# westlake-repl/Adapter4Rec

Measured on NVIDIA B200. Metric: train user-sequences/s (SASRec + BERT-base LoRA r=8 adapter-tuning step: fwd+bwd+allreduce+Adam), higher is better.
Workload: dtype bf16

## Files before the change

### adapter4rec_b200/csrc/attention_mid.cu

```cuda
#include "a4r_common.cuh"
#include "mma_sync.cuh"

namespace {

constexpr int DH = 64;
constexpr int WARPS = 8;
constexpr int LMAX = 256;

A4R_DEVICE uint32_t toff(int row, int chunk) { return static_cast<uint32_t>(row * 128 + (((chunk ^ row) & 7) << 4)); }

struct MidParams {
  const __nv_bfloat16* qkv;
  __nv_bfloat16* out;
  const __nv_bfloat16* dout;
  const void* mask;
  float* lse;
  const __nv_bfloat16* ctx;
  int64_t ld_qkv, ld_out, mask_ld;
  int N, L, Lp, heads;
  int mask_dtype;
  float scale, mask_neg;
};

A4R_DEVICE void load_rows(uint8_t* tile, const __nv_bfloat16* g, int64_t ld, int L, int Lp) {
  const uint32_t base = smem_u32(tile);
  for (int i = threadIdx.x; i < Lp * 8; i += WARPS * 32) {
    const int row = i >> 3, ch = i & 7;
    const bool ok = row < L;
    const __nv_bfloat16* src = g + (ok ? static_cast<int64_t>(row) * ld + ch * 8 : 0);
    const int sz = ok ? 16 : 0;
    asm volatile("cp.async.cg.shared.global [%0], [%1], 16, %2;" ::"r"(base + toff(row, ch)), "l"(src), "r"(sz) : "memory");
  }
}
A4R_DEVICE void cp_async_wait_all() { asm volatile("cp.async.wait_all;" ::: "memory"); }

A4R_DEVICE void lda(uint32_t (&a)[4], uint32_t base, int m0, int k0, int lane) {
  const int mi = lane >> 3, r = lane & 7;
  ldsm_x4(a, base + toff(m0 + r + ((mi & 1) << 3), (k0 >> 3) + (mi >> 1)));
}
A4R_DEVICE void ldb_nk(uint32_t (&b)[4], uint32_t base, int n0, int k0, int lane) {
  const int mi = lane >> 3, r = lane & 7;
  ldsm_x4(b, base + toff(n0 + r + ((mi >> 1) << 3), (k0 >> 3) + (mi & 1)));
}
A4R_DEVICE void ldb_kn(uint32_t (&b)[4], uint32_t base, int n0, int k0, int lane) {
  const int mi = lane >> 3, r = lane & 7;
  ldsm_x4_t(b, base + toff(k0 + r + ((mi & 1) << 3), (n0 >> 3) + (mi >> 1)));
}
A4R_DEVICE void c2a(uint32_t (&a)[4], const float (&c0)[4], const float (&c1)[4]) {
  a[0] = pack_bf16x2(c0[0], c0[1]);
  a[1] = pack_bf16x2(c0[2], c0[3]);
  a[2] = pack_bf16x2(c1[0], c1[1]);
  a[3] = pack_bf16x2(c1[2], c1[3]);
}

A4R_DEVICE bool key_ok(const MidParams& p, int n, int j) {
  if (j >= p.L) return false;
  if (p.mask_dtype == 1) return reinterpret_cast<const int64_t*>(p.mask)[static_cast<int64_t>(n) * p.mask_ld + j] != 0;
  if (p.mask_dtype == 2) return reinterpret_cast<const float*>(p.mask)[static_cast<int64_t>(n) * p.mask_ld + j] != 0.0f;
  return true;
}

A4R_DEVICE void score_block(float (&s)[8][4], const uint32_t (&qa)[4][4], uint32_t sK, int key0, int lane, int nv) {
#pragma unroll
  for (int nt = 0; nt < 8; ++nt)
#pragma unroll
    for (int e = 0; e < 4; ++e) s[nt][e] = 0.0f;
#pragma unroll
  for (int ks = 0; ks < 4; ++ks) {
#pragma unroll
    for (int np = 0; np < 4; ++np) {
      if (np < nv) {
        uint32_t b[4];
        ldb_nk(b, sK, key0 + np * 16, ks * 16, lane);
        const uint32_t b0[2] = {b[0], b[1]}, b1[2] = {b[2], b[3]};
        mma_bf16_16816(s[np * 2], qa[ks], b0);
        mma_bf16_16816(s[np * 2 + 1], qa[ks], b1);
      }
    }
  }
}

A4R_DEVICE void mask_block(float (&s)[8][4], const MidParams& p, const uint32_t* kvalid, int key0, int lane) {
  const int t = lane & 3;
#pragma unroll
  for (int nt = 0; nt < 8; ++nt)
#pragma unroll
    for (int e = 0; e < 4; ++e) {
      const int j = key0 + nt * 8 + 2 * t + (e & 1);
      float v = s[nt][e] * p.scale;
      const bool valid = (kvalid[j >> 5] >> (j & 31)) & 1u;
      if (!valid) v += p.mask_neg;
      if (j >= p.L) v = -INFINITY;
      s[nt][e] = v;
    }
}

__global__ void __launch_bounds__(WARPS * 32, 2) attn_mid_fwd_kernel(const MidParams p) {
  extern __shared__ __align__(128) uint8_t sm_mid[];
  __shared__ uint32_t kvalid[LMAX / 32];
  const int warp = threadIdx.x >> 5, lane = threadIdx.x & 31;
  const int g = lane >> 2, t = lane & 3;
  const int tile_bytes = p.Lp * 128;
  uint8_t *tQ = sm_mid, *tK = sm_mid + tile_bytes, *tV = sm_mid + 2 * tile_bytes;
  const uint32_t sQ = smem_u32(tQ), sK = smem_u32(tK), sV = smem_u32(tV);
  const int64_t Hd = static_cast<int64_t>(p.heads) * DH;
  for (int w = blockIdx.x; w < p.N * p.heads; w += gridDim.x) {
    const int n = w / p.heads, h = w % p.heads;
    const __nv_bfloat16* q = p.qkv + static_cast<int64_t>(n) * p.L * p.ld_qkv + h * DH;
    __syncthreads();
    load_rows(tQ, q, p.ld_qkv, p.L, p.Lp);
    load_rows(tK, q + Hd, p.ld_qkv, p.L, p.Lp);
    load_rows(tV, q + 2 * Hd, p.ld_qkv, p.L, p.Lp);
    if (threadIdx.x < LMAX / 32) {
      uint32_t bits = 0;
      for (int j = 0; j < 32; ++j) bits |= (key_ok(p, n, threadIdx.x * 32 + j) ? 1u : 0u) << j;
      kvalid[threadIdx.x] = bits;
    }
    cp_async_wait_all();
    __syncthreads();
    for (int m0 = warp * 16; m0 < p.Lp && m0 < ((p.L + 15) & ~15); m0 += WARPS * 16) {
      uint32_t qa[4][4];
#pragma unroll
      for (int ks = 0; ks < 4; ++ks) lda(qa[ks], sQ, m0, ks * 16, lane);
      float o[8][4];
#pragma unroll
      for (int nt = 0; nt < 8; ++nt)
#pragma unroll
        for (int e = 0; e < 4; ++e) o[nt][e] = 0.0f;
      float mx[2] = {-INFINITY, -INFINITY}, sum[2] = {0.0f, 0.0f};
      for (int key0 = 0; key0 < p.Lp; key0 += 64) {
        float s[8][4];
        const int nv = min(4, (p.L - key0 + 15) >> 4);
        score_block(s, qa, sK, key0, lane, nv);
        mask_block(s, p, kvalid, key0, lane);
#pragma unroll
        for (int hh = 0; hh < 2; ++hh) {
          float bm = -INFINITY;
#pragma unroll
          for (int nt = 0; nt < 8; ++nt) bm = fmaxf(bm, fmaxf(s[nt][hh * 2], s[nt][hh * 2 + 1]));
          bm = fmaxf(bm, __shfl_xor_sync(0xffffffffu, bm, 1));
          bm = fmaxf(bm, __shfl_xor_sync(0xffffffffu, bm, 2));
          const float nm = fmaxf(mx[hh], bm);
          const float corr = (mx[hh] == -INFINITY) ? 0.0f : __expf(mx[hh] - nm);
          mx[hh] = nm;
          float bs = 0.0f;
#pragma unroll
          for (int nt = 0; nt < 8; ++nt)
#pragma unroll
            for (int e = 0; e < 2; ++e) {
              const float ex = (nm == -INFINITY || (nt >> 1) >= nv) ? 0.0f : __expf(s[nt][hh * 2 + e] - nm);
              s[nt][hh * 2 + e] = ex;
              bs += ex;
            }
          bs += __shfl_xor_sync(0xffffffffu, bs, 1);
          bs += __shfl_xor_sync(0xffffffffu, bs, 2);
          sum[hh] = sum[hh] * corr + bs;
#pragma unroll
          for (int nt = 0; nt < 8; ++nt) {
            o[nt][hh * 2] *= corr;
            o[nt][hh * 2 + 1] *= corr;
          }
        }
#pragma unroll
        for (int ks = 0; ks < 4; ++ks) {
          if (ks < nv) {
            uint32_t a[4];
            c2a(a, s[2 * ks], s[2 * ks + 1]);
#pragma unroll
            for (int np = 0; np < 4; ++np) {
              uint32_t b[4];
              ldb_kn(b, sV, np * 16, key0 + ks * 16, lane);
              const uint32_t b0[2] = {b[0], b[1]}, b1[2] = {b[2], b[3]};
              mma_bf16_16816(o[np * 2], a, b0);
              mma_bf16_16816(o[np * 2 + 1], a, b1);
            }
          }
        }
      }
      const float inv0 = 1.0f / sum[0], inv1 = 1.0f / sum[1];
      __nv_bfloat16* op = p.out + (static_cast<int64_t>(n) * p.L) * p.ld_out + h * DH;
      const int r0 = m0 + g, r1 = m0 + g + 8;
      if (p.lse != nullptr && t == 0) {
        if (r0 < p.L) p.lse[(static_cast<int64_t>(n) * p.L + r0) * p.heads + h] = mx[0] + __logf(sum[0]);
        if (r1 < p.L) p.lse[(static_cast<int64_t>(n) * p.L + r1) * p.heads + h] = mx[1] + __logf(sum[1]);
      }
#pragma unroll
      for (int nt = 0; nt < 8; ++nt) {
        const int col = nt * 8 + 2 * t;
        if (r0 < p.L) *reinterpret_cast<uint32_t*>(op + static_cast<int64_t>(r0) * p.ld_out + col) = pack_bf16x2(o[nt][0] * inv0, o[nt][1] * inv0);
        if (r1 < p.L) *reinterpret_cast<uint32_t*>(op + static_cast<int64_t>(r1) * p.ld_out + col) = pack_bf16x2(o[nt][2] * inv1, o[nt][3] * inv1);
      }
    }
  }
}

__global__ void __launch_bounds__(WARPS * 32) attn_mid_bwd_kernel(const MidParams p) {
  extern __shared__ __align__(128) uint8_t sm_mid[];
  __shared__ uint32_t kvalid[LMAX / 32];
  __shared__ float s_lse[LMAX], s_delta[LMAX];
  const int warp = threadIdx.x >> 5, lane = threadIdx.x & 31;
  const int g = lane >> 2, t = lane & 3;
  const int tile_bytes = p.Lp * 128;
  uint8_t *tQ = sm_mid, *tK = tQ + tile_bytes, *tV = tK + tile_bytes, *tdO = tV + tile_bytes;
  const uint32_t sQ = smem_u32(tQ), sK = smem_u32(tK), sV = smem_u32(tV), sdO = smem_u32(tdO);
  const int64_t Hd = static_cast<int64_t>(p.heads) * DH;
  const int Lq = (p.L + 15) & ~15;
  for (int w = blockIdx.x; w < p.N * p.heads; w += gridDim.x) {
    const int n = w / p.heads, h = w % p.heads;
    const __nv_bfloat16* q = p.qkv + static_cast<int64_t>(n) * p.L * p.ld_qkv + h * DH;
    __nv_bfloat16* dq = p.out + static_cast<int64_t>(n) * p.L * p.ld_qkv + h * DH;
    __syncthreads();
    load_rows(tQ, q, p.ld_qkv, p.L, p.Lp);
    load_rows(tK, q + Hd, p.ld_qkv, p.L, p.Lp);
    load_rows(tV, q + 2 * Hd, p.ld_qkv, p.L, p.Lp);
    load_rows(tdO, p.dout + static_cast<int64_t>(n) * p.L * p.ld_out + h * DH, p.ld_out, p.L, p.Lp);
    if (threadIdx.x < LMAX / 32) {
      uint32_t bits = 0;
      for (int j = 0; j < 32; ++j) bits |= (key_ok(p, n, threadIdx.x * 32 + j) ? 1u : 0u) << j;
      kvalid[threadIdx.x] = bits;
    }
    cp_async_wait_all();
    __syncthreads();
    for (int r = threadIdx.x; r < p.Lp; r += WARPS * 32)
      s_lse[r] = r < p.L ? p.lse[(static_cast<int64_t>(n) * p.L + r) * p.heads + h] : 0.0f;
    for (int i = threadIdx.x; i < p.Lp * 8; i += WARPS * 32) {
      const int r = i >> 3, ch = i & 7;
      float d = 0.0f;
      if (r < p.L) {
        const int64_t grow = static_cast<int64_t>(n) * p.L + r;
        const uint4 ov = ld_nc_v4(p.ctx + grow * p.ld_out + h * DH + ch * 8);
        const uint4 dv4 = *reinterpret_cast<const uint4*>(tdO + toff(r, ch));
        const uint32_t ow[4] = {ov.x, ov.y, ov.z, ov.w}, dw[4] = {dv4.x, dv4.y, dv4.z, dv4.w};
#pragma unroll
        for (int e = 0; e < 4; ++e) {
          const float2 a = unpack_bf16x2(ow[e]), b = unpack_bf16x2(dw[e]);
          d += a.x * b.x + a.y * b.y;
        }
      }
      d += __shfl_xor_sync(0xffffffffu, d, 1);
      d += __shfl_xor_sync(0xffffffffu, d, 2);
      d += __shfl_xor_sync(0xffffffffu, d, 4);
      if (ch == 0) s_delta[r] = d;
    }
    __syncthreads();
    for (int m0 = warp * 16; m0 < Lq; m0 += WARPS * 16) {
      uint32_t qa[4][4], da[4][4];
#pragma unroll
      for (int ks = 0; ks < 4; ++ks) {
        lda(qa[ks], sQ, m0, ks * 16, lane);
        lda(da[ks], sdO, m0, ks * 16, lane);
      }
      const float lse[2] = {s_lse[m0 + g], s_lse[m0 + g + 8]};
      const float delta[2] = {s_delta[m0 + g], s_delta[m0 + g + 8]};
      float acc[8][4];
#pragma unroll
      for (int nt = 0; nt < 8; ++nt)
#pragma unroll
        for (int e = 0; e < 4; ++e) acc[nt][e] = 0.0f;
      for (int key0 = 0; key0 < p.Lp; key0 += 64) {
        float s[8][4], dp[8][4];
        const int nv = min(4, (p.L - key0 + 15) >> 4);
        score_block(s, qa, sK, key0, lane, nv);
        mask_block(s, p, kvalid, key0, lane);
        score_block(dp, da, sV, key0, lane, nv);
#pragma unroll
        for (int nt = 0; nt < 8; ++nt)
          if ((nt >> 1) < nv) {
#pragma unroll
            for (int e = 0; e < 4; ++e)
              s[nt][e] = __expf(s[nt][e] - lse[e >> 1]) * (dp[nt][e] - delta[e >> 1]) * p.scale;
          }
#pragma unroll
        for (int ks = 0; ks < 4; ++ks) {
          if (ks < nv) {
            uint32_t a[4];
            c2a(a, s[2 * ks], s[2 * ks + 1]);
#pragma unroll
            for (int np = 0; np < 4; ++np) {
              uint32_t b[4];
              ldb_kn(b, sK, np * 16, key0 + ks * 16, lane);
              const uint32_t b0[2] = {b[0], b[1]}, b1[2] = {b[2], b[3]};
              mma_bf16_16816(acc[np * 2], a, b0);
              mma_bf16_16816(acc[np * 2 + 1], a, b1);
            }
          }
        }
      }
      const int r0 = m0 + g, r1 = m0 + g + 8;
#pragma unroll
      for (int nt = 0; nt < 8; ++nt) {
        const int col = nt * 8 + 2 * t;
        if (r0 < p.L) *reinterpret_cast<uint32_t*>(dq + static_cast<int64_t>(r0) * p.ld_qkv + col) = pack_bf16x2(acc[nt][0], acc[nt][1]);
        if (r1 < p.L) *reinterpret_cast<uint32_t*>(dq + static_cast<int64_t>(r1) * p.ld_qkv + col) = pack_bf16x2(acc[nt][2], acc[nt][3]);
      }
    }
    for (int j0 = warp * 16; j0 < Lq; j0 += WARPS * 16) {
      uint32_t ka[4][4], va[4][4];
#pragma unroll
      for (int ks = 0; ks < 4; ++ks) {
        lda(ka[ks], sK, j0, ks * 16, lane);
        lda(va[ks], sV, j0, ks * 16, lane);
      }
      const int jr[2] = {j0 + g, j0 + g + 8};
      bool kv[2];
#pragma unroll
      for (int hh = 0; hh < 2; ++hh) kv[hh] = (kvalid[jr[hh] >> 5] >> (jr[hh] & 31)) & 1u;
      float dk[8][4], dv[8][4];
#pragma unroll
      for (int nt = 0; nt < 8; ++nt)
#pragma unroll
        for (int e = 0; e < 4; ++e) dk[nt][e] = dv[nt][e] = 0.0f;
      for (int i0 = 0; i0 < p.Lp; i0 += 64) {
        float st[8][4], dpt[8][4];
        const int nv = min(4, (p.L - i0 + 15) >> 4);
        score_block(st, ka, sQ, i0, lane, nv);
        score_block(dpt, va, sdO, i0, lane, nv);
#pragma unroll
        for (int nt = 0; nt < 8; ++nt)
#pragma unroll
          for (int e = 0; e < 4; ++e) {
            const int i = i0 + nt * 8 + 2 * t + (e & 1);
            const int hh = e >> 1;
            float v = st[nt][e] * p.scale;
            if (!kv[hh]) v += p.mask_neg;
            float pr = 0.0f, ds = 0.0f;
            if (jr[hh] < p.L && i < p.L) {
              pr = __expf(v - s_lse[i]);
              ds = pr * (dpt[nt][e] - s_delta[i]) * p.scale;
            }
            st[nt][e] = pr;
            dpt[nt][e] = ds;
          }
#pragma unroll
        for (int ks = 0; ks < 4; ++ks) {
          if (ks >= nv) continue;
          uint32_t pa[4], sa[4];
          c2a(pa, st[2 * ks], st[2 * ks + 1]);
          c2a(sa, dpt[2 * ks], dpt[2 * ks + 1]);
#pragma unroll
          for (int np = 0; np < 4; ++np) {
            uint32_t b[4], c[4];
            ldb_kn(b, sQ, np * 16, i0 + ks * 16, lane);
            ldb_kn(c, sdO, np * 16, i0 + ks * 16, lane);
            const uint32_t b0[2] = {b[0], b[1]}, b1[2] = {b[2], b[3]};
            const uint32_t c0[2] = {c[0], c[1]}, c1[2] = {c[2], c[3]};
            mma_bf16_16816(dk[np * 2], sa, b0);
            mma_bf16_16816(dk[np * 2 + 1], sa, b1);
            mma_bf16_16816(dv[np * 2], pa, c0);
            mma_bf16_16816(dv[np * 2 + 1], pa, c1);
          }
        }
      }
#pragma unroll
      for (int nt = 0; nt < 8; ++nt) {
        const int col = nt * 8 + 2 * t;
#pragma unroll
        for (int hh = 0; hh < 2; ++hh) {
          if (jr[hh] < p.L) {
            __nv_bfloat16* row = dq + static_cast<int64_t>(jr[hh]) * p.ld_qkv + col;
            *reinterpret_cast<uint32_t*>(row + Hd) = pack_bf16x2(dk[nt][hh * 2], dk[nt][hh * 2 + 1]);
            *reinterpret_cast<uint32_t*>(row + 2 * Hd) = pack_bf16x2(dv[nt][hh * 2], dv[nt][hh * 2 + 1]);
          }
        }
      }
    }
  }
}

constexpr float LOG2E = 1.4426950408889634f;


int check_mid(const a4r_attn_args* a) {
  A4R_CHECK_ARG(a != nullptr && a->qkv && a->out, "attention_mid: NULL pointer");
  A4R_CHECK_ARG(a->L >= 1 && a->L <= LMAX, "attention_mid: L must be in [1,256] (got %lld)", (long long)a->L);
  A4R_CHECK_ARG(a->head_dim == DH, "attention_mid: head_dim must be 64");
  A4R_CHECK_ARG(a->causal == 0, "attention_mid: causal masking is not supported (use the short-sequence kernel)");
  A4R_CHECK_ARG(a->dropout_p == 0.0f, "attention_mid: probability dropout is not implemented (ViT uses p = 0)");
  A4R_CHECK_ARG(a->heads >= 1 && a->N >= 0, "attention_mid: bad heads/N");
  A4R_CHECK_ARG(a->ld_qkv >= 3 * a->heads * DH && a->ld_qkv % 8 == 0 && a->ld_out >= a->heads * DH && a->ld_out % 8 == 0,
                "attention_mid: bad leading dimensions");
  A4R_CHECK_ARG(a4r_aligned16(a->qkv) && a4r_aligned16(a->out), "attention_mid: pointers must be 16B aligned");
  A4R_CHECK_ARG(a->mask_dtype >= 0 && a->mask_dtype <= 2, "attention_mid: mask_dtype must be 0,1,2");
  if (a->mask_dtype != 0) A4R_CHECK_ARG(a->mask != nullptr && a->mask_ld >= a->L, "attention_mid: bad mask");
  return a4r_device_check();
}

MidParams mid_params(const a4r_attn_args* a) {
  MidParams p;
  p.qkv = static_cast<const __nv_bfloat16*>(a->qkv);
  p.out = static_cast<__nv_bfloat16*>(a->out);
  p.dout = static_cast<const __nv_bfloat16*>(a->dout);
  p.mask = a->mask;
  p.lse = a->lse;
  p.ctx = static_cast<const __nv_bfloat16*>(a->ctx);
  p.ld_qkv = a->ld_qkv;
  p.ld_out = a->ld_out;
  p.mask_ld = a->mask_ld;
  p.N = static_cast<int>(a->N);
  p.L = static_cast<int>(a->L);
  p.Lp = (p.L + 63) & ~63;
  p.heads = static_cast<int>(a->heads);
  p.mask_dtype = a->mask_dtype;
  p.scale = a->scale;
  p.mask_neg = a->mask_neg;
  return p;
}

}

int a4r_attn_vit_tc_fwd(const a4r_attn_args* a, cudaStream_t stream);
int a4r_attn_vit_tc_bwd(const a4r_attn_args* a, cudaStream_t stream);

extern "C" int a4r_attn_mid_fwd(const a4r_attn_args* a, a4r_stream_t stream) {
  int rc = check_mid(a);
  if (rc != A4R_OK) return rc;
  if (a->N == 0) return A4R_OK;
  if (a->mask_dtype == 0) return a4r_attn_vit_tc_fwd(a, static_cast<cudaStream_t>(stream));
  const MidParams p = mid_params(a);
  const int smem = 3 * p.Lp * 128;
  A4R_CUDA_OK(cudaFuncSetAttribute(attn_mid_fwd_kernel, cudaFuncAttributeMaxDynamicSharedMemorySize, 3 * LMAX * 128));
  int64_t blocks = static_cast<int64_t>(p.N) * p.heads;
  const int64_t cap = static_cast<int64_t>(a4r_num_sms()) * 4;
  if (blocks > cap) blocks = cap;
  attn_mid_fwd_kernel<<<static_cast<int>(blocks), WARPS * 32, smem, static_cast<cudaStream_t>(stream)>>>(p);
  A4R_LAUNCH_OK();
  a4r_count_launch(1);
  return A4R_OK;
}

extern "C" int a4r_attn_mid_bwd(const a4r_attn_args* a, a4r_stream_t stream) {
  int rc = check_mid(a);
  if (rc != A4R_OK) return rc;
  A4R_CHECK_ARG(a->dout != nullptr && a4r_aligned16(a->dout), "attention_mid bwd: dout missing or unaligned");
  A4R_CHECK_ARG(a->lse != nullptr && a->ctx != nullptr, "attention_mid bwd: needs the forward's lse and ctx outputs");
  if (a->N == 0) return A4R_OK;
  if (a->mask_dtype == 0) return a4r_attn_vit_tc_bwd(a, static_cast<cudaStream_t>(stream));
  const MidParams p = mid_params(a);
  const int smem = 4 * p.Lp * 128;
  A4R_CUDA_OK(cudaFuncSetAttribute(attn_mid_bwd_kernel, cudaFuncAttributeMaxDynamicSharedMemorySize, 4 * LMAX * 128));
  int64_t blocks = static_cast<int64_t>(p.N) * p.heads;
  const int64_t cap = static_cast<int64_t>(a4r_num_sms()) * 2;
  if (blocks > cap) blocks = cap;
  attn_mid_bwd_kernel<<<static_cast<int>(blocks), WARPS * 32, smem, static_cast<cudaStream_t>(stream)>>>(p);
  A4R_LAUNCH_OK();
  a4r_count_launch(1);
  return A4R_OK;
}
```

### adapter4rec_b200/csrc/attention_small.cu

```cuda
#include "a4r_common.cuh"
#include "mma_sync.cuh"

namespace {

constexpr int LP = 32;
constexpr int WARPS_PER_CTA = 4;

struct AttnParams {
  const __nv_bfloat16* qkv;
  __nv_bfloat16* out;
  const __nv_bfloat16* dout;
  const void* mask;
  int64_t ld_qkv, ld_out, mask_ld;
  int N, L, heads;
  int mask_dtype;
  const int32_t* cu_seqlens;
  int causal;
  float scale, mask_neg;
  uint32_t drop_thr16;
  float drop_scale;
  uint64_t drop_seed, drop_offset;
};

A4R_DEVICE void prob_dropout(float (&s)[2][4][4], const AttnParams& p, int n, int h, int lane) {
  const int g = lane >> 2, t = lane & 3;
  const uint64_t base = p.drop_offset + (static_cast<uint64_t>(n) * p.heads + h) * (32 * 8);
  const uint64_t seed = rng_seed(p.drop_seed);
#pragma unroll
  for (int mt = 0; mt < 2; ++mt)
#pragma unroll
    for (int hh = 0; hh < 2; ++hh) {
      const int i = mt * 16 + hh * 8 + g;
#pragma unroll
      for (int np = 0; np < 2; ++np) {
        const uint64_t r = rng64(seed, base + static_cast<uint64_t>(i) * 8 + np * 4 + t);
#pragma unroll
        for (int q = 0; q < 2; ++q)
#pragma unroll
          for (int e = 0; e < 2; ++e) {
            float& x = s[mt][np * 2 + q][hh * 2 + e];
            x = rng_keep(r, q * 2 + e, p.drop_thr16) ? x * p.drop_scale : 0.0f;
          }
      }
    }
}

template <int COLS>
struct Tile {
  static constexpr int kChunks = COLS / 8;
  static constexpr int kBytes = LP * COLS * 2;
  A4R_DEVICE static uint32_t off(int row, int chunk) {
    const int x = COLS == 64 ? row : (row >> 1);
    return static_cast<uint32_t>(row * COLS * 2 + (((chunk ^ x) & (kChunks - 1)) << 4));
  }
};

template <int COLS>
A4R_DEVICE void load_a(uint32_t (&a)[4], uint32_t base, int m0, int k0, int lane) {
  const int mi = lane >> 3, r = lane & 7;
  const int row = m0 + r + ((mi & 1) << 3);
  const int chunk = (k0 >> 3) + (mi >> 1);
  ldsm_x4(a, base + Tile<COLS>::off(row, chunk));
}
template <int COLS>
A4R_DEVICE void load_a_t(uint32_t (&a)[4], uint32_t base, int m0, int k0, int lane) {
  const int mi = lane >> 3, r = lane & 7;
  const int row = k0 + r + ((mi >> 1) << 3);
  const int chunk = (m0 >> 3) + (mi & 1);
  ldsm_x4_t(a, base + Tile<COLS>::off(row, chunk));
}
template <int COLS>
A4R_DEVICE void load_b_nk(uint32_t (&b)[4], uint32_t base, int n0, int k0, int lane) {
  const int mi = lane >> 3, r = lane & 7;
  const int row = n0 + r + ((mi >> 1) << 3);
  const int chunk = (k0 >> 3) + (mi & 1);
  ldsm_x4(b, base + Tile<COLS>::off(row, chunk));
}
template <int COLS>
A4R_DEVICE void load_b_kn(uint32_t (&b)[4], uint32_t base, int n0, int k0, int lane) {
  const int mi = lane >> 3, r = lane & 7;
  const int row = k0 + r + ((mi & 1) << 3);
  const int chunk = (n0 >> 3) + (mi >> 1);
  ldsm_x4_t(b, base + Tile<COLS>::off(row, chunk));
}

template <int DH>
A4R_DEVICE void load_tile(uint8_t* tile, const __nv_bfloat16* g, int64_t ld, int L, int lane) {
  constexpr int CH = DH / 8;
  const uint32_t base = smem_u32(tile);
#pragma unroll
  for (int i = lane; i < LP * CH; i += 32) {
    const int row = i / CH, ch = i % CH;
    const bool ok = row < L;
    const __nv_bfloat16* src = g + (ok ? static_cast<int64_t>(row) * ld + ch * 8 : 0);
    const int sz = ok ? 16 : 0;
    asm volatile("cp.async.cg.shared.global [%0], [%1], 16, %2;" ::"r"(base + Tile<DH>::off(row, ch)), "l"(src), "r"(sz)
                 : "memory");
  }
}
A4R_DEVICE void cp_async_wait_all() { asm volatile("cp.async.wait_all;" ::: "memory"); }
template <int DH>
A4R_DEVICE void store_tile(const uint8_t* tile, __nv_bfloat16* g, int64_t ld, int L, int lane) {
  constexpr int CH = DH / 8;
#pragma unroll
  for (int i = lane; i < LP * CH; i += 32) {
    const int row = i / CH, ch = i % CH;
    if (row < L) st_na_v4(g + static_cast<int64_t>(row) * ld + ch * 8, *reinterpret_cast<const uint4*>(tile + Tile<DH>::off(row, ch)));
  }
}
template <int COLS, int NT>
A4R_DEVICE void acc_to_tile(uint8_t* tile, const float (&acc)[2][NT][4], float s0a, float s0b, float s1a, float s1b, int lane) {
  const int g = lane >> 2, t = lane & 3;
#pragma unroll
  for (int mt = 0; mt < 2; ++mt) {
    const float sa = mt == 0 ? s0a : s1a, sb = mt == 0 ? s0b : s1b;
#pragma unroll
    for (int nt = 0; nt < NT; ++nt) {
      const int r0 = mt * 16 + g, col = nt * 8 + 2 * t;
      *reinterpret_cast<uint32_t*>(tile + Tile<COLS>::off(r0, col >> 3) + (col & 7) * 2) =
          pack_bf16x2(acc[mt][nt][0] * sa, acc[mt][nt][1] * sa);
      *reinterpret_cast<uint32_t*>(tile + Tile<COLS>::off(r0 + 8, col >> 3) + (col & 7) * 2) =
          pack_bf16x2(acc[mt][nt][2] * sb, acc[mt][nt][3] * sb);
    }
  }
}

struct SeqSpan {
  int64_t row0, mask0;
  int L;
};
A4R_DEVICE SeqSpan seq_span(const AttnParams& p, int n) {
  SeqSpan s;
  if (p.cu_seqlens != nullptr) {
    const int a = __ldg(p.cu_seqlens + n), b = __ldg(p.cu_seqlens + n + 1);
    s.row0 = a, s.mask0 = a, s.L = b - a;
  } else {
    s.row0 = static_cast<int64_t>(n) * p.L, s.mask0 = static_cast<int64_t>(n) * p.mask_ld, s.L = p.L;
  }
  return s;
}
A4R_DEVICE bool key_valid(const AttnParams& p, const SeqSpan& sq, int j) {
  if (p.mask_dtype == 1) return reinterpret_cast<const int64_t*>(p.mask)[sq.mask0 + j] != 0;
  if (p.mask_dtype == 2) return reinterpret_cast<const float*>(p.mask)[sq.mask0 + j] != 0.0f;
  return true;
}

template <int DH>
A4R_DEVICE void scores_softmax(float (&s)[2][4][4], uint32_t sQ, uint32_t sK, const AttnParams& p, int L, int lane,
                               uint32_t keymask_bits) {
#pragma unroll
  for (int mt = 0; mt < 2; ++mt)
#pragma unroll
    for (int nt = 0; nt < 4; ++nt)
#pragma unroll
      for (int e = 0; e < 4; ++e) s[mt][nt][e] = 0.0f;
#pragma unroll
  for (int k0 = 0; k0 < DH; k0 += 16) {
    uint32_t a0[4], a1[4];
    load_a<DH>(a0, sQ, 0, k0, lane);
    load_a<DH>(a1, sQ, 16, k0, lane);
#pragma unroll
    for (int np = 0; np < 2; ++np) {
      uint32_t b[4];
      load_b_nk<DH>(b, sK, np * 16, k0, lane);
      const uint32_t b0[2] = {b[0], b[1]}, b1[2] = {b[2], b[3]};
      mma_bf16_16816(s[0][np * 2], a0, b0);
      mma_bf16_16816(s[0][np * 2 + 1], a0, b1);
      mma_bf16_16816(s[1][np * 2], a1, b0);
      mma_bf16_16816(s[1][np * 2 + 1], a1, b1);
    }
  }
  const int g = lane >> 2, t = lane & 3;
  float colneg[4][2];
#pragma unroll
  for (int nt = 0; nt < 4; ++nt)
#pragma unroll
    for (int e = 0; e < 2; ++e) {
      const int j = nt * 8 + 2 * t + e;
      colneg[nt][e] = j >= L ? -INFINITY : (((keymask_bits >> j) & 1u) ? 0.0f : p.mask_neg);
    }
#pragma unroll
  for (int mt = 0; mt < 2; ++mt) {
#pragma unroll
    for (int h = 0; h < 2; ++h) {
      const int i = mt * 16 + h * 8 + g;
      float mx = -INFINITY;
#pragma unroll
      for (int nt = 0; nt < 4; ++nt)
#pragma unroll
        for (int e = 0; e < 2; ++e) {
          float v = fmaf(s[mt][nt][h * 2 + e], p.scale, colneg[nt][e]);
          if (p.causal && nt * 8 + 2 * t + e > i && colneg[nt][e] == 0.0f) v += p.mask_neg;
          s[mt][nt][h * 2 + e] = v;
          mx = fmaxf(mx, v);
        }
      mx = fmaxf(mx, __shfl_xor_sync(0xffffffffu, mx, 1));
      mx = fmaxf(mx, __shfl_xor_sync(0xffffffffu, mx, 2));
      float sum = 0.0f;
#pragma unroll
      for (int nt = 0; nt < 4; ++nt)
#pragma unroll
        for (int e = 0; e < 2; ++e) {
          const float ex = __expf(s[mt][nt][h * 2 + e] - mx);
          s[mt][nt][h * 2 + e] = ex;
          sum += ex;
        }
      sum += __shfl_xor_sync(0xffffffffu, sum, 1);
      sum += __shfl_xor_sync(0xffffffffu, sum, 2);
      const float inv = 1.0f / sum;
#pragma unroll
      for (int nt = 0; nt < 4; ++nt)
#pragma unroll
        for (int e = 0; e < 2; ++e) s[mt][nt][h * 2 + e] *= inv;
    }
  }
}

A4R_DEVICE uint32_t build_keymask(const AttnParams& p, const SeqSpan& sq, int lane) {
  const bool ok = lane < sq.L ? key_valid(p, sq, lane) : false;
  return __ballot_sync(0xffffffffu, ok);
}

A4R_DEVICE void acc_to_a(uint32_t (&a)[4], const float (&c0)[4], const float (&c1)[4]) {
  a[0] = pack_bf16x2(c0[0], c0[1]);
  a[1] = pack_bf16x2(c0[2], c0[3]);
  a[2] = pack_bf16x2(c1[0], c1[1]);
  a[3] = pack_bf16x2(c1[2], c1[3]);
}

template <int DH>
__global__ void __launch_bounds__(WARPS_PER_CTA * 32, 3) attn_fwd_kernel(const AttnParams p) {
  extern __shared__ __align__(128) uint8_t smem_attn[];
  constexpr int TB = Tile<DH>::kBytes;
  const int warp = threadIdx.x >> 5, lane = threadIdx.x & 31;
  uint8_t* my = smem_attn + warp * 3 * TB;
  const int64_t total = static_cast<int64_t>(p.N) * p.heads;
  for (int64_t w = static_cast<int64_t>(blockIdx.x) * WARPS_PER_CTA + warp; w < total;
       w += static_cast<int64_t>(gridDim.x) * WARPS_PER_CTA) {
    const int n = static_cast<int>(w / p.heads), h = static_cast<int>(w % p.heads);
    const int64_t Hd = static_cast<int64_t>(p.heads) * DH;
    const SeqSpan sq = seq_span(p, n);
    const __nv_bfloat16* q = p.qkv + sq.row0 * p.ld_qkv + h * DH;
    load_tile<DH>(my, q, p.ld_qkv, sq.L, lane);
    load_tile<DH>(my + TB, q + Hd, p.ld_qkv, sq.L, lane);
    load_tile<DH>(my + 2 * TB, q + 2 * Hd, p.ld_qkv, sq.L, lane);
    const uint32_t km = build_keymask(p, sq, lane);
    cp_async_wait_all();
    __syncwarp();
    const uint32_t sQ = smem_u32(my), sK = sQ + TB, sV = sK + TB;
    float s[2][4][4];
    scores_softmax<DH>(s, sQ, sK, p, sq.L, lane, km);
    if (p.drop_thr16 != 0) prob_dropout(s, p, n, h, lane);
    float o[2][DH / 8][4];
#pragma unroll
    for (int mt = 0; mt < 2; ++mt)
#pragma unroll
      for (int nt = 0; nt < DH / 8; ++nt)
#pragma unroll
        for (int e = 0; e < 4; ++e) o[mt][nt][e] = 0.0f;
#pragma unroll
    for (int ks = 0; ks < 2; ++ks) {
      uint32_t a0[4], a1[4];
      acc_to_a(a0, s[0][2 * ks], s[0][2 * ks + 1]);
      acc_to_a(a1, s[1][2 * ks], s[1][2 * ks + 1]);
#pragma unroll
      for (int np = 0; np < DH / 16; ++np) {
        uint32_t b[4];
        load_b_kn<DH>(b, sV, np * 16, ks * 16, lane);
        const uint32_t b0[2] = {b[0], b[1]}, b1[2] = {b[2], b[3]};
        mma_bf16_16816(o[0][np * 2], a0, b0);
        mma_bf16_16816(o[0][np * 2 + 1], a0, b1);
        mma_bf16_16816(o[1][np * 2], a1, b0);
        mma_bf16_16816(o[1][np * 2 + 1], a1, b1);
      }
    }
    __syncwarp();
    acc_to_tile<DH, DH / 8>(my, o, 1.f, 1.f, 1.f, 1.f, lane);
    __syncwarp();
    store_tile<DH>(my, p.out + sq.row0 * p.ld_out + h * DH, p.ld_out, sq.L, lane);
    __syncwarp();
  }
}

template <int DH>
__global__ void __launch_bounds__(WARPS_PER_CTA * 32) attn_bwd_kernel(const AttnParams p) {
  extern __shared__ __align__(128) uint8_t smem_attn[];
  constexpr int TB = Tile<DH>::kBytes;
  constexpr int PB = Tile<32>::kBytes;
  const int warp = threadIdx.x >> 5, lane = threadIdx.x & 31;
  uint8_t* my = smem_attn + warp * (4 * TB + 2 * PB);
  const int64_t total = static_cast<int64_t>(p.N) * p.heads;
  for (int64_t w = static_cast<int64_t>(blockIdx.x) * WARPS_PER_CTA + warp; w < total;
       w += static_cast<int64_t>(gridDim.x) * WARPS_PER_CTA) {
    const int n = static_cast<int>(w / p.heads), h = static_cast<int>(w % p.heads);
    const int64_t Hd = static_cast<int64_t>(p.heads) * DH;
    const SeqSpan sq = seq_span(p, n);
    const __nv_bfloat16* q = p.qkv + sq.row0 * p.ld_qkv + h * DH;
    uint8_t *tQ = my, *tK = my + TB, *tV = my + 2 * TB, *tdO = my + 3 * TB, *tP = my + 4 * TB, *tdS = tP + PB;
    load_tile<DH>(tQ, q, p.ld_qkv, sq.L, lane);
    load_tile<DH>(tK, q + Hd, p.ld_qkv, sq.L, lane);
    load_tile<DH>(tV, q + 2 * Hd, p.ld_qkv, sq.L, lane);
    load_tile<DH>(tdO, p.dout + sq.row0 * p.ld_out + h * DH, p.ld_out, sq.L, lane);
    const uint32_t km = build_keymask(p, sq, lane);
    cp_async_wait_all();
    __syncwarp();
    const uint32_t sQ = smem_u32(tQ), sK = smem_u32(tK), sV = smem_u32(tV), sdO = smem_u32(tdO), sP = smem_u32(tP),
                   sdS = smem_u32(tdS);
    float s[2][4][4];
    scores_softmax<DH>(s, sQ, sK, p, sq.L, lane, km);
    float dp[2][4][4];
#pragma unroll
    for (int mt = 0; mt < 2; ++mt)
#pragma unroll
      for (int nt = 0; nt < 4; ++nt)
#pragma unroll
        for (int e = 0; e < 4; ++e) dp[mt][nt][e] = 0.0f;
#pragma unroll
    for (int k0 = 0; k0 < DH; k0 += 16) {
      uint32_t a0[4], a1[4];
      load_a<DH>(a0, sdO, 0, k0, lane);
      load_a<DH>(a1, sdO, 16, k0, lane);
#pragma unroll
      for (int np = 0; np < 2; ++np) {
        uint32_t b[4];
        load_b_nk<DH>(b, sV, np * 16, k0, lane);
        const uint32_t b0[2] = {b[0], b[1]}, b1[2] = {b[2], b[3]};
        mma_bf16_16816(dp[0][np * 2], a0, b0);
        mma_bf16_16816(dp[0][np * 2 + 1], a0, b1);
        mma_bf16_16816(dp[1][np * 2], a1, b0);
        mma_bf16_16816(dp[1][np * 2 + 1], a1, b1);
      }
    }
    float sd[2][4][4];
#pragma unroll
    for (int mt = 0; mt < 2; ++mt)
#pragma unroll
      for (int nt = 0; nt < 4; ++nt)
#pragma unroll
        for (int e = 0; e < 4; ++e) sd[mt][nt][e] = s[mt][nt][e];
    if (p.drop_thr16 != 0) {
      prob_dropout(sd, p, n, h, lane);
#pragma unroll
      for (int mt = 0; mt < 2; ++mt)
#pragma unroll
        for (int nt = 0; nt < 4; ++nt)
#pragma unroll
          for (int e = 0; e < 4; ++e) dp[mt][nt][e] = (sd[mt][nt][e] != 0.0f) ? dp[mt][nt][e] * p.drop_scale : 0.0f;
    }
#pragma unroll
    for (int mt = 0; mt < 2; ++mt)
#pragma unroll
      for (int hh = 0; hh < 2; ++hh) {
        float d = 0.0f;
#pragma unroll
        for (int nt = 0; nt < 4; ++nt)
#pragma unroll
          for (int e = 0; e < 2; ++e) d += s[mt][nt][hh * 2 + e] * dp[mt][nt][hh * 2 + e];
        d += __shfl_xor_sync(0xffffffffu, d, 1);
        d += __shfl_xor_sync(0xffffffffu, d, 2);
#pragma unroll
        for (int nt = 0; nt < 4; ++nt)
#pragma unroll
          for (int e = 0; e < 2; ++e)
            dp[mt][nt][hh * 2 + e] = s[mt][nt][hh * 2 + e] * (dp[mt][nt][hh * 2 + e] - d) * p.scale;
      }
    acc_to_tile<32, 4>(tP, sd, 1.f, 1.f, 1.f, 1.f, lane);
    acc_to_tile<32, 4>(tdS, dp, 1.f, 1.f, 1.f, 1.f, lane);
    __syncwarp();
    float acc[2][DH / 8][4];
#pragma unroll
    for (int mt = 0; mt < 2; ++mt)
#pragma unroll
      for (int nt = 0; nt < DH / 8; ++nt)
#pragma unroll
        for (int e = 0; e < 4; ++e) acc[mt][nt][e] = 0.0f;
#pragma unroll
    for (int ks = 0; ks < 2; ++ks) {
      uint32_t a0[4], a1[4];
      acc_to_a(a0, dp[0][2 * ks], dp[0][2 * ks + 1]);
      acc_to_a(a1, dp[1][2 * ks], dp[1][2 * ks + 1]);
#pragma unroll
      for (int np = 0; np < DH / 16; ++np) {
        uint32_t b[4];
        load_b_kn<DH>(b, sK, np * 16, ks * 16, lane);
        const uint32_t b0[2] = {b[0], b[1]}, b1[2] = {b[2], b[3]};
        mma_bf16_16816(acc[0][np * 2], a0, b0);
        mma_bf16_16816(acc[0][np * 2 + 1], a0, b1);
        mma_bf16_16816(acc[1][np * 2], a1, b0);
        mma_bf16_16816(acc[1][np * 2 + 1], a1, b1);
      }
    }
    float dk[2][DH / 8][4], dv[2][DH / 8][4];
#pragma unroll
    for (int mt = 0; mt < 2; ++mt)
#pragma unroll
      for (int nt = 0; nt < DH / 8; ++nt)
#pragma unroll
        for (int e = 0; e < 4; ++e) dk[mt][nt][e] = dv[mt][nt][e] = 0.0f;
#pragma unroll
    for (int ks = 0; ks < 2; ++ks) {
      uint32_t a0[4], a1[4], p0[4], p1[4];
      load_a_t<32>(a0, sdS, 0, ks * 16, lane);
      load_a_t<32>(a1, sdS, 16, ks * 16, lane);
      load_a_t<32>(p0, sP, 0, ks * 16, lane);
      load_a_t<32>(p1, sP, 16, ks * 16, lane);
#pragma unroll
      for (int np = 0; np < DH / 16; ++np) {
        uint32_t b[4];
        load_b_kn<DH>(b, sQ, np * 16, ks * 16, lane);
        const uint32_t b0[2] = {b[0], b[1]}, b1[2] = {b[2], b[3]};
        mma_bf16_16816(dk[0][np * 2], a0, b0);
        mma_bf16_16816(dk[0][np * 2 + 1], a0, b1);
        mma_bf16_16816(dk[1][np * 2], a1, b0);
        mma_bf16_16816(dk[1][np * 2 + 1], a1, b1);
        uint32_t c[4];
        load_b_kn<DH>(c, sdO, np * 16, ks * 16, lane);
        const uint32_t c0[2] = {c[0], c[1]}, c1[2] = {c[2], c[3]};
        mma_bf16_16816(dv[0][np * 2], p0, c0);
        mma_bf16_16816(dv[0][np * 2 + 1], p0, c1);
        mma_bf16_16816(dv[1][np * 2], p1, c0);
        mma_bf16_16816(dv[1][np * 2 + 1], p1, c1);
      }
    }
    __syncwarp();
    acc_to_tile<DH, DH / 8>(tQ, acc, 1.f, 1.f, 1.f, 1.f, lane);
    acc_to_tile<DH, DH / 8>(tK, dk, 1.f, 1.f, 1.f, 1.f, lane);
    acc_to_tile<DH, DH / 8>(tV, dv, 1.f, 1.f, 1.f, 1.f, lane);
    __syncwarp();
    __nv_bfloat16* dq = p.out + sq.row0 * p.ld_qkv + h * DH;
    store_tile<DH>(tQ, dq, p.ld_qkv, sq.L, lane);
    store_tile<DH>(tK, dq + Hd, p.ld_qkv, sq.L, lane);
    store_tile<DH>(tV, dq + 2 * Hd, p.ld_qkv, sq.L, lane);
    __syncwarp();
  }
}

int check_common(const a4r_attn_args* a) {
  A4R_CHECK_ARG(a != nullptr, "attention: args is NULL");
  A4R_CHECK_ARG(a->qkv && a->out, "attention: qkv/out must be non-NULL");
  A4R_CHECK_ARG(a->L >= 1 && a->L <= LP, "attention_small: L must be in [1,32] (got %lld)", (long long)a->L);
  A4R_CHECK_ARG(a->head_dim == 32 || a->head_dim == 64, "attention_small: head_dim must be 32 or 64");
  A4R_CHECK_ARG(a->heads >= 1 && a->N >= 0, "attention: bad heads/N");
  A4R_CHECK_ARG(a->ld_qkv >= 3 * a->heads * a->head_dim && a->ld_qkv % 8 == 0, "attention: bad ld_qkv");
  A4R_CHECK_ARG(a->ld_out >= a->heads * a->head_dim && a->ld_out % 8 == 0, "attention: bad ld_out");
  A4R_CHECK_ARG(a4r_aligned16(a->qkv) && a4r_aligned16(a->out), "attention: pointers must be 16B aligned");
  A4R_CHECK_ARG(a->mask_dtype >= 0 && a->mask_dtype <= 2, "attention: mask_dtype must be 0,1,2");
  if (a->mask_dtype != 0)
    A4R_CHECK_ARG(a->mask != nullptr && (a->cu_seqlens != nullptr || a->mask_ld >= a->L), "attention: bad mask/mask_ld");
  A4R_CHECK_ARG(a->dropout_p >= 0.0f && a->dropout_p < 1.0f, "attention: dropout_p must be in [0,1)");
  return a4r_device_check();
}

AttnParams to_params(const a4r_attn_args* a) {
  AttnParams p;
  p.qkv = static_cast<const __nv_bfloat16*>(a->qkv);
  p.out = static_cast<__nv_bfloat16*>(a->out);
  p.dout = static_cast<const __nv_bfloat16*>(a->dout);
  p.mask = a->mask;
  p.ld_qkv = a->ld_qkv;
  p.ld_out = a->ld_out;
  p.mask_ld = a->mask_ld;
  p.N = static_cast<int>(a->N);
  p.L = static_cast<int>(a->L);
  p.cu_seqlens = a->cu_seqlens;
  p.heads = static_cast<int>(a->heads);
  p.mask_dtype = a->mask_dtype;
  p.causal = a->causal;
  p.scale = a->scale;
  p.mask_neg = a->mask_neg;
  p.drop_thr16 = static_cast<uint32_t>(a->dropout_p * 65536.0f + 0.5f);
  p.drop_scale = 65536.0f / static_cast<float>(65536u - p.drop_thr16);
  p.drop_seed = a->dropout_seed;
  p.drop_offset = a->dropout_offset;
  return p;
}

template <typename K>
int launch(K kernel, int smem, const AttnParams& p, cudaStream_t stream, bool* attr_done) {
  if (!*attr_done) {
    A4R_CUDA_OK(cudaFuncSetAttribute(kernel, cudaFuncAttributeMaxDynamicSharedMemorySize, smem));
    *attr_done = true;
  }
  const int64_t total = static_cast<int64_t>(p.N) * p.heads;
  int64_t blocks = (total + WARPS_PER_CTA - 1) / WARPS_PER_CTA;
  const int64_t cap = static_cast<int64_t>(a4r_num_sms()) * 8;
  if (blocks > cap) blocks = cap;
  kernel<<<static_cast<int>(blocks), WARPS_PER_CTA * 32, smem, stream>>>(p);
  A4R_LAUNCH_OK();
  a4r_count_launch(1);
  return A4R_OK;
}

}

extern "C" int a4r_attn_small_fwd(const a4r_attn_args* a, a4r_stream_t stream) {
  int rc = check_common(a);
  if (rc != A4R_OK) return rc;
  if (a->N == 0) return A4R_OK;
  const AttnParams p = to_params(a);
  static bool done64 = false, done32 = false;
  if (a->head_dim == 64)
    return launch(attn_fwd_kernel<64>, WARPS_PER_CTA * 3 * Tile<64>::kBytes, p, static_cast<cudaStream_t>(stream), &done64);
  return launch(attn_fwd_kernel<32>, WARPS_PER_CTA * 3 * Tile<32>::kBytes, p, static_cast<cudaStream_t>(stream), &done32);
}

extern "C" int a4r_attn_small_bwd(const a4r_attn_args* a, a4r_stream_t stream) {
  int rc = check_common(a);
  if (rc != A4R_OK) return rc;
  A4R_CHECK_ARG(a->dout != nullptr && a4r_aligned16(a->dout), "attention bwd: dout missing or unaligned");
  if (a->N == 0) return A4R_OK;
  const AttnParams p = to_params(a);
  static bool done64 = false, done32 = false;
  if (a->head_dim == 64)
    return launch(attn_bwd_kernel<64>, WARPS_PER_CTA * (4 * Tile<64>::kBytes + 2 * Tile<32>::kBytes), p,
                  static_cast<cudaStream_t>(stream), &done64);
  return launch(attn_bwd_kernel<32>, WARPS_PER_CTA * (4 * Tile<32>::kBytes + 2 * Tile<32>::kBytes), p,
                static_cast<cudaStream_t>(stream), &done32);
}
```

### adapter4rec_b200/functional.py

```python
import torch

from . import ops

BF16 = torch.bfloat16


PARAM_EPOCH = [0]


def bump_param_epoch():
    PARAM_EPOCH[0] += 1


class WeightCache:

    def __init__(self):
        self.key = None
        self.master = None
        self.w = None
        self.wt = None

    def get(self, weight, need_t=False):
        key = (weight.data_ptr(), weight._version, weight.device, PARAM_EPOCH[0] if weight.requires_grad else -1)
        if key != self.key:
            self.key = key
            self.master = weight.detach()
            if self._fusable(self.master):
                self.w, self.wt = ops.cast_transpose(self.master, True, need_t)
            else:
                self.w, self.wt = self.master.to(BF16).contiguous(), None
        if need_t and self.wt is None:
            if self._fusable(self.master):
                _, self.wt = ops.cast_transpose(self.master, False, True)
            else:
                self.wt = self.w.t().contiguous()
        return self.w, self.wt

    @staticmethod
    def _fusable(w):
        return w.is_cuda and w.dtype == torch.float32 and w.dim() == 2 and w.stride(1) == 1


def _as2d(x):
    return x.reshape(-1, x.shape[-1])


class LinearFunction(torch.autograd.Function):

    @staticmethod
    def forward(ctx, x, weight, bias, residual, residual2, cache, act):
        w, _ = cache.get(weight)
        standalone = act in ("leaky_relu", "gelu_new")
        epi = {None: ops.EPI_LINEAR, "gelu": ops.EPI_GELU, "relu": ops.EPI_RELU}[None if standalone else act]
        b = None if bias is None else bias.detach().float().contiguous()
        need_grad = any(ctx.needs_input_grad[:5])
        aux = None
        if act == "gelu" and need_grad:
            aux = torch.empty((x.shape[0], w.shape[0]), dtype=BF16, device=x.device)
        y = ops.gemm(x, w, bias=b, epilogue=epi, residual=residual, residual2=residual2, aux=aux)
        if standalone:
            aux, y = y, ops.act_fwd(y, act)
        ctx.cache, ctx.act = cache, act
        ctx.has_bias, ctx.has_r1, ctx.has_r2 = bias is not None, residual is not None, residual2 is not None
        save_x = x if ctx.needs_input_grad[1] else None
        act_saved = aux if act in ("gelu", "gelu_new") else (y if act in ("relu", "leaky_relu") else None)
        ctx.save_for_backward(save_x, act_saved, weight)
        return y

    @staticmethod
    def backward(ctx, dy):
        x, act_saved, weight = ctx.saved_tensors
        dy = dy.contiguous()
        if ctx.act is not None:
            dy = ops.act_bwd(dy, act_saved, ctx.act)
        dx = dw = db = None
        if ctx.needs_input_grad[0]:
            _, wt = ctx.cache.get(weight, need_t=True)
            dx = ops.gemm(dy, wt)
        if ctx.needs_input_grad[1]:
            dw = ops.wgrad(dy, x)
        if ctx.has_bias and ctx.needs_input_grad[2]:
            db = ops.colsum(dy)
        dr1 = dy if ctx.has_r1 and ctx.needs_input_grad[3] else None
        dr2 = dy if ctx.has_r2 and ctx.needs_input_grad[4] else None
        return dx, dw, db, dr1, dr2, None, None


def linear(x, weight, bias, cache, act=None, residual=None, residual2=None):
    assert act is None or (residual is None and residual2 is None)
    return LinearFunction.apply(x, weight, bias, residual, residual2, cache, act)


class FFNFunction(torch.autograd.Function):

    @staticmethod
    def forward(ctx, y, wi, bi, wf, bf, residual, cache_i, cache_f):
        w1, _ = cache_i.get(wi)
        w2, _ = cache_f.get(wf)
        need = ctx.needs_input_grad[0] or ctx.needs_input_grad[5]
        u = torch.empty((y.shape[0], w1.shape[0]), dtype=BF16, device=y.device) if need else None
        f = ops.gemm(y, w1, bias=bi.detach(), epilogue=ops.EPI_GELU, aux=u)
        h = ops.gemm(f, w2, bias=bf.detach(), residual=residual)
        ctx.caches = (cache_i, cache_f)
        ctx.has_res = residual is not None
        ctx.res_is_input = residual is y
        ctx.save_for_backward(u, wi, wf)
        return h

    @staticmethod
    def backward(ctx, dh):
        u, wi, wf = ctx.saved_tensors
        dh = dh.contiguous()
        _, w2t = ctx.caches[1].get(wf, need_t=True)
        _, w1t = ctx.caches[0].get(wi, need_t=True)
        du = ops.gemm(dh, w2t, epilogue=ops.EPI_DGELU, aux=u)
        fold = ctx.has_res and ctx.res_is_input
        dy = ops.gemm(du, w1t, residual=dh if fold else None) if ctx.needs_input_grad[0] else None
        dres = dh if (ctx.has_res and not fold and ctx.needs_input_grad[5]) else None
        return dy, None, None, None, None, dres, None, None


class PostLNBlockFunction(torch.autograd.Function):

    @staticmethod
    def forward(ctx, x, res, gamma, beta, eps, p, w1, b1, cache1, w2, b2, cache2):
        ffn = w2 is not None
        need = any(ctx.needs_input_grad[:4])
        rng = (float(p),) + DropoutState.draw((x.shape[0] * (w2 if ffn else w1).shape[0] + 3) // 4) if p > 0 else None
        wa, _ = cache1.get(w1)
        u = None
        if ffn:
            wb, _ = cache2.get(w2)
            u = torch.empty((x.shape[0], wa.shape[0]), dtype=BF16, device=x.device) if need else None
            f = ops.gemm(x, wa, bias=b1.detach(), epilogue=ops.EPI_GELU, aux=u)
            z = ops.gemm(f, wb, bias=b2.detach(), residual=res, dropout=rng)
        else:
            z = ops.gemm(x, wa, bias=b1.detach(), residual=res, dropout=rng)
        g, b = gamma.detach().float().contiguous(), beta.detach().float().contiguous()
        out, _, mean, rstd = ops.layernorm_fwd(z, g, b, eps, want_stats=need)
        ctx.rng, ctx.ffn, ctx.caches = rng, ffn, (cache1, cache2)
        ctx.res_is_input = res is x
        if need:
            ctx.save_for_backward(z, mean, rstd, g, u, w1, w2)
        return out

    @staticmethod
    def backward(ctx, dout):
        z, mean, rstd, g, u, w1, w2 = ctx.saved_tensors
        dout = dout.contiguous()
        want_ln = ctx.needs_input_grad[2] or ctx.needs_input_grad[3]
        dg = db = None
        if want_ln:
            dg, db = torch.empty_like(g), torch.empty_like(g)
        r = ops.layernorm_bwd(dout, z, mean, rstd, g, dgamma=dg, dbeta=db, masked=ctx.rng)
        dz, dzm = r if ctx.rng is not None else (r, r)
        dx = None
        if ctx.needs_input_grad[0]:
            fold = dz if ctx.res_is_input else None
            if ctx.ffn:
                _, w2t = ctx.caches[1].get(w2, need_t=True)
                _, w1t = ctx.caches[0].get(w1, need_t=True)
                du = ops.gemm(dzm, w2t, epilogue=ops.EPI_DGELU, aux=u)
                dx = ops.gemm(du, w1t, residual=fold)
            else:
                _, w1t = ctx.caches[0].get(w1, need_t=True)
                dx = ops.gemm(dzm, w1t, residual=fold)
        dres = dz if (ctx.needs_input_grad[1] and not ctx.res_is_input) else None
        return dx, dres, dg, db, None, None, None, None, None, None, None, None


class LayerNormFunction(torch.autograd.Function):

    @staticmethod
    def forward(ctx, x, weight, bias, eps, res, res_param=None):
        need = any(ctx.needs_input_grad[:3]) or (res_param is not None and res_param.requires_grad)
        g, b = weight.detach().float().contiguous(), bias.detach().float().contiguous()
        if res is not None:
            y, z, mean, rstd = ops.layernorm_fwd(x, g, b, eps, res=res, want_z=need, want_stats=need)
        else:
            y, _, mean, rstd = ops.layernorm_fwd(x, g, b, eps, want_stats=need)
            z = x
        ctx.res_rows = 0 if res is None else res.numel() // res.shape[-1]
        ctx.res_shape = None if res_param is None else tuple(res_param.shape)
        if need:
            ctx.save_for_backward(z, mean, rstd, g)
        return y

    @staticmethod
    def backward(ctx, dy):
        z, mean, rstd, g = ctx.saved_tensors
        dy = dy.contiguous()
        dg = db = None
        if ctx.needs_input_grad[1] or ctx.needs_input_grad[2]:
            dg, db = torch.empty_like(g), torch.empty_like(g)
        dz = ops.layernorm_bwd(dy, z, mean, rstd, g, dgamma=dg, dbeta=db)
        dres = None
        if ctx.res_shape is not None and ctx.needs_input_grad[5]:
            rows, H = ctx.res_rows, dz.shape[1]
            dres = torch.zeros(ctx.res_shape, dtype=torch.float32, device=dz.device)
            dres[:rows] = ops.colsum(dz.view(-1, rows * H)).view(rows, H)
        return dz, dg, db, None, None, dres


def layer_norm(x, weight, bias, eps, res=None, res_param=None):
    return LayerNormFunction.apply(x, weight, bias, eps, res, res_param)


class LayerNormSkipFunction(torch.autograd.Function):

    @staticmethod
    def forward(ctx, x, weight, bias, eps):
        need = any(ctx.needs_input_grad[:3])
        g, b = weight.detach().float().contiguous(), bias.detach().float().contiguous()
        y, _, mean, rstd = ops.layernorm_fwd(x, g, b, eps, want_stats=need)
        if need:
            ctx.save_for_backward(x, mean, rstd, g)
        return y, x

    @staticmethod
    def backward(ctx, dy, dskip):
        x, mean, rstd, g = ctx.saved_tensors
        want_ln = ctx.needs_input_grad[1] or ctx.needs_input_grad[2]
        if dy is None:
            return dskip, None, None, None
        dy = dy.contiguous()
        if dskip is not None and not want_ln:
            return ops.layernorm_bwd_add(dy, x, mean, rstd, g, dskip.contiguous()), None, None, None
        dg = db = None
        if want_ln:
            dg, db = torch.empty_like(g), torch.empty_like(g)
        dx = ops.layernorm_bwd(dy, x, mean, rstd, g, dgamma=dg, dbeta=db)
        if dskip is not None:
            dx = dx + dskip
        return dx, dg, db, None


def layer_norm_skip(x, weight, bias, eps):
    return LayerNormSkipFunction.apply(x, weight, bias, eps)


class DropoutState:
    seed = 0x5EEDA4D2
    counter = 0
    seed_address = None
    SEED_INDIRECT = 1 << 63

    @classmethod
    def manual_seed(cls, seed):
        cls.seed, cls.counter = int(seed) & 0xFFFFFFFFFFFF, 0

    @classmethod
    def draw(cls, n_counters):
        off = cls.counter
        cls.counter += int(n_counters)
        if cls.seed_address is not None:
            return cls.SEED_INDIRECT | int(cls.seed_address), off
        return cls.seed, off

    @classmethod
    def replay_seed(cls, step, base=None):
        z = ((cls.seed if base is None else int(base)) + 0x9E3779B97F4A7C15 * (int(step) + 1)) & 0xFFFFFFFFFFFFFFFF
        z = ((z ^ (z >> 30)) * 0xBF58476D1CE4E5B9) & 0xFFFFFFFFFFFFFFFF
        z = ((z ^ (z >> 27)) * 0x94D049BB133111EB) & 0xFFFFFFFFFFFFFFFF
        return (z ^ (z >> 31)) & 0x7FFFFFFFFFFFFFFF


class DropoutAddFunction(torch.autograd.Function):

    @staticmethod
    def forward(ctx, x, res, p):
        ctx.p = p
        ctx.rng = DropoutState.draw((x.numel() + 3) // 4)
        ctx.has_res = res is not None
        return ops.dropout(x.contiguous(), None if res is None else res.contiguous(), p, *ctx.rng)

    @staticmethod
    def backward(ctx, dy):
        dy = dy.contiguous()
        dx = ops.dropout(dy, None, ctx.p, *ctx.rng) if ctx.needs_input_grad[0] else None
        return dx, (dy if ctx.has_res and ctx.needs_input_grad[1] else None), None


def dropout_add(x, res, p):
    return DropoutAddFunction.apply(x, res, float(p))


class AddFunction(torch.autograd.Function):

    @staticmethod
    def forward(ctx, x, res):
        return ops.dropout(x.contiguous(), res.contiguous(), 0.0, 0, 0)

    @staticmethod
    def backward(ctx, dy):
        return (dy if ctx.needs_input_grad[0] else None), (dy if ctx.needs_input_grad[1] else None)


def add(x, res):
    return AddFunction.apply(x, res)


class AttentionFunction(torch.autograd.Function):
    @staticmethod
    def forward(ctx, qkv, mask, N, L, heads, head_dim, causal, mask_neg, dropout_p=0.0, scale=None, cu_seqlens=None):
        ctx.cfg = (N, L, heads, head_dim, causal, mask_neg, scale)
        ctx.cu = cu_seqlens
        ctx.mask = mask
        ctx.drop = None
        if dropout_p > 0.0:
            ctx.drop = (dropout_p,) + DropoutState.draw(N * heads * 32 * 8)
        out, lse = ops.attn_small_fwd(qkv, N, L, heads, head_dim, mask=mask, causal=causal, mask_neg=mask_neg, want_lse=True,
                                      dropout=ctx.drop, scale=scale, cu_seqlens=cu_seqlens)
        ctx.save_for_backward(qkv, lse, out if lse is not None else None)
        return out

    @staticmethod
    def backward(ctx, dctx):
        qkv, lse, out = ctx.saved_tensors
        N, L, heads, head_dim, causal, mask_neg, scale = ctx.cfg
        dqkv = ops.attn_small_bwd(qkv, dctx.contiguous(), N, L, heads, head_dim, mask=ctx.mask, causal=causal,
                                  mask_neg=mask_neg, lse=lse, ctx=out, dropout=ctx.drop, scale=scale, cu_seqlens=ctx.cu)
        return dqkv, None, None, None, None, None, None, None, None, None, None


def attention(qkv, mask, N, L, heads, head_dim, causal=False, mask_neg=ops.F32_MIN, dropout_p=0.0, scale=None,
              cu_seqlens=None):
    return AttentionFunction.apply(qkv, mask, N, L, heads, head_dim, causal, mask_neg, float(dropout_p), scale, cu_seqlens)


class GatherRowsFunction(torch.autograd.Function):

    @staticmethod
    def forward(ctx, x, idx):
        ctx.rows = x.shape[0]
        ctx.save_for_backward(idx)
        return ops.gather_rows(x.contiguous(), idx)

    @staticmethod
    def backward(ctx, dy):
        (idx,) = ctx.saved_tensors
        dx = torch.zeros((ctx.rows, dy.shape[1]), dtype=dy.dtype, device=dy.device)
        dx.index_copy_(0, idx, dy.contiguous())
        return dx, None


def gather_rows(x, idx):
    return GatherRowsFunction.apply(x, idx)


class ExpandRowsFunction(torch.autograd.Function):

    @staticmethod
    def forward(ctx, x, inverse, counts):
        ctx.save_for_backward(inverse, counts)
        return ops.gather_rows(x.contiguous(), inverse)

    @staticmethod
    def backward(ctx, dy):
        inverse, counts = ctx.saved_tensors
        order = torch.argsort(inverse, stable=True)
        grouped = dy.contiguous()[order].float()
        return torch.segment_reduce(grouped, "sum", lengths=counts, axis=0).to(dy.dtype), None, None


def expand_rows(x, inverse, counts):
    return ExpandRowsFunction.apply(x, inverse, counts)


_ROW_HASH = {}


def unique_rows(rows):
    N, W = rows.shape
    key = (rows.device, W)
    if key not in _ROW_HASH:
        g = torch.Generator().manual_seed(0x5EED)
        _ROW_HASH[key] = (torch.randint(-2 ** 62, 2 ** 62, (W,), generator=g, dtype=torch.int64) | 1).to(rows.device)
    h = (rows * _ROW_HASH[key]).sum(1)
    uh, inverse, counts = torch.unique(h, return_inverse=True, return_counts=True)
    first = torch.full((uh.numel(),), N, dtype=torch.int64, device=rows.device)
    first.scatter_reduce_(0, inverse, torch.arange(N, device=rows.device), reduce="amin")
    uniq = rows[first]
    if not bool((uniq[inverse] == rows).all()):
        uniq, inverse, counts = torch.unique(rows, dim=0, return_inverse=True, return_counts=True)
    return uniq, inverse, counts


LORA_PAD = 64


class QKVFunction(torch.autograd.Function):

    @staticmethod
    def forward(ctx, x, cache, *params):
        ctx.with_skip = len(params) > 0 and isinstance(params[-1], str) and params[-1] == "skip"
        if ctx.with_skip:
            params = params[:-1]
        ctx.set_materialize_grads(False)
        assert len(params) % 4 == 0
        n = len(params) // 4
        H = params[0].shape[0]
        K = params[0].shape[1]
        dev = x.device
        frozen_w = not any(p is not None and p.requires_grad for p in [params[4 * j] for j in range(n)])
        key = tuple((p.data_ptr(), p._version) for p in [params[4 * j] for j in range(n)]) + (PARAM_EPOCH[0] if not frozen_w else -1,)
        if cache.get("key") != key or not frozen_w:
            cache["key"] = key
            cache["w"] = torch.cat([params[i].detach().to(BF16) for i in range(0, 4 * n, 4)], 0).contiguous()
            cache["wt"] = None
        w = cache["w"]
        small = [params[4 * j + i] for j in range(n) for i in (1, 2, 3)]
        skey = (PARAM_EPOCH[0],) + tuple(None if p is None else (p.data_ptr(), p._version) for p in small)
        reuse = cache.get("small_key") == skey
        if reuse:
            bias = cache["bias"]
        else:
            zero_h = cache.get("zero_h")
            if zero_h is None or zero_h.device != dev or zero_h.numel() != H:
                zero_h = cache["zero_h"] = torch.zeros(H, dtype=torch.float32, device=dev)
            bias = torch.cat([zero_h if params[4 * j + 1] is None else params[4 * j + 1].detach().float() for j in range(n)])
            cache["small_key"], cache["bias"] = skey, bias
        slots, off = [], 0
        for j in range(n):
            A = params[4 * j + 2]
            if A is not None:
                r = A.shape[0]
                slots.append((j, off, r))
                off += r
        assert off <= LORA_PAD, "sum of LoRA ranks of one fused projection must be <= 64"
        T = a_cat = b_ext = None
        if slots:
            ctx.ones_col = off < LORA_PAD
            if reuse and "a_cat" in cache:
                a_cat, b_ext, t_bias = cache["a_cat"], cache["b_ext"], cache["t_bias"]
            else:
                st = cache.get("lora_stage")
                if st is None or st[0].device != dev or st[0].shape != (LORA_PAD, K) or st[1].shape != (n * H, LORA_PAD):
                    st = cache["lora_stage"] = (torch.zeros((LORA_PAD, K), dtype=torch.float32, device=dev),
                                                torch.zeros((n * H, LORA_PAD), dtype=torch.float32, device=dev))
                    cache["lora_slots"] = None
                if cache.get("lora_slots") != slots:
                    st[0].zero_()
                    st[1].zero_()
                    cache["lora_slots"] = list(slots)
                for j, o, r in slots:
                    st[0][o:o + r].copy_(params[4 * j + 2].detach())
                    torch.mul(params[4 * j + 3].detach(), 1.0 / r, out=st[1][j * H:(j + 1) * H, o:o + r])
                a_cat, a_cat_t = ops.cast_transpose(st[0], True, True)
                b_ext, b_ext_t = ops.cast_transpose(st[1], True, True)
                tb = cache.get("t_bias_const")
                if tb is None or tb[0] != ctx.ones_col or tb[1].device != dev:
                    t_bias = torch.zeros(LORA_PAD, dtype=torch.float32, device=dev)
                    if ctx.ones_col:
                        t_bias[LORA_PAD - 1] = 1.0
                    tb = cache["t_bias_const"] = (ctx.ones_col, t_bias)
                t_bias = tb[1]
                cache["a_cat"], cache["b_ext"], cache["t_bias"] = a_cat, b_ext, t_bias
                cache["a_cat_t"], cache["b_ext_t"] = a_cat_t, b_ext_t
            T = ops.gemm(x, a_cat, bias=t_bias)
            qkv = ops.gemm(x, w, bias=bias, a2=T, b2=b_ext)
        else:
            qkv = ops.gemm(x, w, bias=bias)
        ctx.cache, ctx.slots, ctx.H, ctx.n = cache, slots, H, n
        if not slots:
            ctx.ones_col = False
        ctx.n_params = len(params)
        ctx.param_needs = [p is not None and p.requires_grad for p in params]
        need_x = any(ctx.param_needs[4 * j + 2] for j in range(n)) or any(ctx.param_needs[4 * j] for j in range(n))
        ctx.save_for_backward(x if need_x else None, T, a_cat, b_ext)
        if ctx.with_skip:
            return qkv, x
        return qkv

    @staticmethod
    def backward(ctx, dqkv, dskip=None):
        x, T, a_cat, b_ext = ctx.saved_tensors
        H, cache, n = ctx.H, ctx.cache, ctx.n
        tail = (None,) if ctx.with_skip else ()
        if dqkv is None:
            return (dskip, None) + (None,) * ctx.n_params + tail
        dqkv = dqkv.contiguous()
        if dskip is not None:
            dskip = dskip.contiguous()
        if cache.get("wt") is None:
            cache["wt"] = cache["w"].t().contiguous()
        grads = [None] * ctx.n_params
        dT = None
        if ctx.slots:
            if cache.get("b_ext") is b_ext and cache.get("b_ext_t") is not None:
                b_ext_t, a_cat_t = cache["b_ext_t"], cache["a_cat_t"]
            else:
                b_ext_t, a_cat_t = b_ext.t().contiguous(), a_cat.t().contiguous()
                if cache.get("b_ext") is b_ext:
                    cache["b_ext_t"], cache["a_cat_t"] = b_ext_t, a_cat_t
            lj = [j for j, _, _ in ctx.slots]
            if n == 3 and len(lj) == 2:
                (ja, jb) = lj
                dT = ops.gemm(dqkv[:, ja * H:(ja + 1) * H], b_ext_t[:, ja * H:(ja + 1) * H],
                              a2=dqkv[:, jb * H:(jb + 1) * H], b2=b_ext_t[:, jb * H:(jb + 1) * H])
            elif n == 3 and len(lj) == 1:
                dT = ops.gemm(dqkv[:, lj[0] * H:(lj[0] + 1) * H], b_ext_t[:, lj[0] * H:(lj[0] + 1) * H])
            else:
                dT = ops.gemm(dqkv, b_ext_t)
            dx = ops.gemm(dqkv, cache["wt"], a2=dT, b2=a_cat_t, residual=dskip) if ctx.needs_input_grad[0] else None
        else:
            dx = ops.gemm(dqkv, cache["wt"], residual=dskip) if ctx.needs_input_grad[0] else None
        fused = bool(ctx.slots) and ctx.ones_col
        if fused:
            want_g1 = any(ctx.param_needs[4 * j + 1] for j in range(n)) or any(ctx.param_needs[4 * j + 3] for j, _, _ in ctx.slots)
            want_g2 = any(ctx.param_needs[4 * j + 2] for j, _, _ in ctx.slots)
            g1_rows = [ctx.param_needs[4 * j + 1] or any(jj == j and ctx.param_needs[4 * j + 3] for jj, _, _ in ctx.slots)
                       for j in range(n)]
            g1 = [None] * n
            if want_g1:
                if all(g1_rows):
                    full = ops.wgrad(dqkv, T)
                    g1 = [full[j * H:(j + 1) * H] for j in range(n)]
                else:
                    g1 = [ops.wgrad(dqkv[:, j * H:(j + 1) * H], T) if g1_rows[j] else None for j in range(n)]
            g2 = ops.wgrad(dT, x) if want_g2 else None
        for j in range(n):
            dq = dqkv[:, j * H:(j + 1) * H]
            if ctx.param_needs[4 * j]:
                grads[4 * j] = ops.wgrad(dq, x)
            if ctx.param_needs[4 * j + 1]:
                grads[4 * j + 1] = g1[j][:, LORA_PAD - 1].contiguous() if fused else ops.colsum(dq)
        for j, o, r in ctx.slots:
            dq = dqkv[:, j * H:(j + 1) * H]
            if ctx.param_needs[4 * j + 3]:
                grads[4 * j + 3] = (g1[j][:, o:o + r] * (1.0 / r)) if fused else \
                    _pad_cols_wgrad(dq, T, o, r, 1.0 / r, transpose=False)
            if ctx.param_needs[4 * j + 2]:
                grads[4 * j + 2] = g2[o:o + r].contiguous() if fused else _pad_cols_wgrad(dT, x, o, r, 1.0, transpose=True)
        return (dx, None) + tuple(grads) + tail


def _pad_cols_wgrad(a, b, off, r, alpha, transpose):
    lo = (off // 8) * 8
    hi = ((off + r + 7) // 8) * 8
    if transpose:
        full = ops.wgrad(a[:, lo:hi], b, alpha=alpha)
        return full[off - lo:off - lo + r].contiguous()
    full = ops.wgrad(a, b[:, lo:hi], alpha=alpha)
    return full[:, off - lo:off - lo + r].contiguous()


class EmbedLNFunction(torch.autograd.Function):

    @staticmethod
    def forward(ctx, ids, L, tables, gamma, beta, eps, roberta_pad_id, prompt, word_pad_idx, *params):
        word, pos, typ = tables
        need_prompt = prompt is not None and prompt.requires_grad
        need_tab = [p is not None and p.requires_grad for p in params] + [False] * (5 - len(params))
        need = need_prompt or any(need_tab)
        p16 = None if prompt is None else prompt.detach().to(BF16).contiguous()
        out, z, mean, rstd = ops.embed_ln_fwd(ids, L, word, pos, typ, gamma, beta, eps, roberta_pad_id=roberta_pad_id,
                                              prompt=p16, want_z=need)
        ctx.L, ctx.need_prompt, ctx.need_tab, ctx.roberta_pad_id, ctx.word_pad_idx = L, need_prompt, need_tab, roberta_pad_id, word_pad_idx
        ctx.n_prompt = 0 if prompt is None else prompt.shape[0]
        ctx.shapes = [None if p is None else tuple(p.shape) for p in params]
        if need:
            ctx.save_for_backward(z, mean, rstd, gamma, ids)
        return out

    @staticmethod
    def backward(ctx, dout):
        z, mean, rstd, gamma, ids = ctx.saved_tensors
        need_word, need_pos, need_typ, need_g, need_b = ctx.need_tab
        dg = db = None
        if need_g or need_b:
            dg, db = torch.empty_like(gamma), torch.empty_like(gamma)
        dz = ops.layernorm_bwd(dout.contiguous(), z, mean, rstd, gamma, dgamma=dg, dbeta=db)
        H = dz.shape[1]
        L, n = ctx.L, ctx.n_prompt
        dp = None
        if ctx.need_prompt:
            dp = ops.colsum(dz.view(-1, L * H), width=n * H).view(n, H)
        grads = [None] * len(ctx.shapes)
        tok = ids[:, :L]
        if need_word:
            idx = tok.clone()
            if n > 0:
                idx[:, :n] = -1
            grads[0] = ops.scatter_add_rows(dz, idx, ctx.shapes[0][0], skip_idx=ctx.word_pad_idx)
        if need_pos:
            P = ctx.shapes[1][0]
            if ctx.roberta_pad_id >= 0:
                m = (tok != ctx.roberta_pad_id).long()
                pos_ids = torch.cumsum(m, 1) * m + ctx.roberta_pad_id
                grads[1] = ops.scatter_add_rows(dz, pos_ids, P, skip_idx=ctx.roberta_pad_id)
            else:
                g = torch.zeros((P, H), dtype=torch.float32, device=dz.device)
                g[:L] = ops.colsum(dz.view(-1, L * H)).view(L, H)
                grads[1] = g
        if need_typ:
            g = torch.zeros(ctx.shapes[2], dtype=torch.float32, device=dz.device)
            g[0] = ops.colsum(dz)
            grads[2] = g
        if need_g:
            grads[3] = dg
        if need_b and len(grads) > 4:
            grads[4] = db
        return (None, None, None, None, None, None, None, dp, None) + tuple(grads)


class BceLossFunction(torch.autograd.Function):
    @staticmethod
    def forward(ctx, prec, emb, log_mask, cpc):
        loss, count, pos, neg = ops.bce_loss_fwd(prec, emb, log_mask, cpc=cpc)
        ctx.cpc = cpc
        ctx.log_mask = log_mask
        ctx.save_for_backward(prec, emb, pos, neg, count)
        return loss.view(())

    @staticmethod
    def backward(ctx, grad_out):
        prec, emb, pos, neg, count = ctx.saved_tensors
        go = grad_out.reshape(1).float().contiguous()
        d_prec, d_emb = ops.bce_loss_bwd(prec, emb, ctx.log_mask, pos, neg, count, grad_out=go, cpc=ctx.cpc)
        return d_prec, d_emb, None, None


def bce_loss(prec, emb, log_mask, cpc=False):
    return BceLossFunction.apply(prec, emb, log_mask, cpc)


class InbatchCeFunction(torch.autograd.Function):

    @staticmethod
    def forward(ctx, prec, emb, item_ids, log_mask, cand_bias):
        loss, count, lse = ops.inbatch_ce_fwd(prec, emb, item_ids, log_mask, cand_bias)
        ctx.aux = (item_ids, log_mask, cand_bias)
        ctx.save_for_backward(prec, emb, lse, count)
        return loss.view(())

    @staticmethod
    def backward(ctx, grad_out):
        prec, emb, lse, count = ctx.saved_tensors
        item_ids, log_mask, cand_bias = ctx.aux
        go = grad_out.reshape(1).float().contiguous()
        d_prec, d_emb = ops.inbatch_ce_bwd(prec, emb, item_ids, log_mask, lse, count, cand_bias=cand_bias, grad_out=go)
        return d_prec, d_emb, None, None, None


def inbatch_softmax_loss(prec, emb, item_ids, log_mask, cand_bias=None):
    return InbatchCeFunction.apply(prec, emb, item_ids, log_mask, cand_bias)


class HoulsbyBlockFunction(torch.autograd.Function):

    @staticmethod
    def forward(ctx, h, inp, w_down, b_down, w_up, b_up, gamma, beta, eps, act, cache_d, cache_u):
        wd, _ = cache_d.get(w_down)
        wu, _ = cache_u.get(w_up)
        tail = 0 if gamma is not None else (1 if inp is not None else 2)
        need = any(ctx.needs_input_grad[:8])
        g = b = None
        if tail == 0:
            g, b = gamma.detach().float().contiguous(), beta.detach().float().contiguous()
        out, z, mean, rstd, s, u = ops.adapter_ln_fwd(h, inp, wd, b_down.detach().float().contiguous(), wu,
                                                      b_up.detach().float().contiguous(), g, b, eps, act=act, tail=tail,
                                                      save=need)
        ctx.act, ctx.tail, ctx.caches, ctx.has_inp = act, tail, (cache_d, cache_u), inp is not None
        if need:
            ctx.save_for_backward(h, z, mean, rstd, g, s, u, w_down, w_up)
        return out

    @staticmethod
    def backward(ctx, dout):
        h, z, mean, rstd, g, s, u, w_down, w_up = ctx.saved_tensors
        dout = dout.contiguous()
        dg = db = None
        if ctx.tail == 0:
            if ctx.needs_input_grad[6] or ctx.needs_input_grad[7]:
                dg, db = torch.empty_like(g), torch.empty_like(g)
            dz = ops.layernorm_bwd(dout, z, mean, rstd, g, dgamma=dg, dbeta=db)
        else:
            dz = dout
        _, wut = ctx.caches[1].get(w_up, need_t=True)
        _, wdt = ctx.caches[0].get(w_down, need_t=True)
        if ctx.act == "gelu":
            ds = ops.gemm(dz, wut, epilogue=ops.EPI_DGELU, aux=u)
        else:
            ds = ops.gemm(dz, wut, epilogue=ops.EPI_DRELU, aux=s)
        dh = ops.gemm(ds, wdt, residual=dz) if ctx.needs_input_grad[0] else None
        dwd = ops.wgrad(ds, h) if ctx.needs_input_grad[2] else None
        dbd = ops.colsum(ds) if ctx.needs_input_grad[3] else None
        dwu = dbu = None
        if ctx.needs_input_grad[4] or ctx.needs_input_grad[5]:
            full = ops.wgrad(dz, ops.s_ext(s))
            dwu, dbu = full[:, :s.shape[1]], full[:, s.shape[1]]
        dinp = dz if (ctx.has_inp and ctx.needs_input_grad[1]) else None
        return dh, dinp, dwd, dbd, dwu, dbu, dg, db, None, None, None, None


def houlsby_block(h, inp, adapter_down, adapter_up, act, ln=None):
    return HoulsbyBlockFunction.apply(h, inp, adapter_down.weight, adapter_down.bias, adapter_up.weight, adapter_up.bias,
                                      None if ln is None else ln.weight, None if ln is None else ln.bias,
                                      0.0 if ln is None else ln.eps, act, adapter_down._cache, adapter_up._cache)


class HoulsbyPostLNBlockFunction(torch.autograd.Function):

    @staticmethod
    def forward(ctx, x, inp, p, w1, b1, cache1, w2, b2, cache2, w_down, b_down, w_up, b_up, gamma, beta, eps, act,
                cache_d, cache_u):
        ffn = w2 is not None
        need = ctx.needs_input_grad[0] or ctx.needs_input_grad[1] or any(ctx.needs_input_grad[9:15])
        wa, _ = cache1.get(w1)
        n_out = (w2 if ffn else w1).shape[0]
        rng = (float(p),) + DropoutState.draw((x.shape[0] * n_out + 3) // 4) if p > 0 else None
        u = None
        if ffn:
            wb, _ = cache2.get(w2)
            u = torch.empty((x.shape[0], wa.shape[0]), dtype=BF16, device=x.device) if need else None
            f = ops.gemm(x, wa, bias=b1.detach(), epilogue=ops.EPI_GELU, aux=u)
            h = ops.gemm(f, wb, bias=b2.detach(), dropout=rng)
        else:
            h = ops.gemm(x, wa, bias=b1.detach(), dropout=rng)
        wd, _ = cache_d.get(w_down)
        wu, _ = cache_u.get(w_up)
        g, b = gamma.detach().float().contiguous(), beta.detach().float().contiguous()
        out, z, mean, rstd, s, u_ad = ops.adapter_ln_fwd(h, inp, wd, b_down.detach().float().contiguous(), wu,
                                                         b_up.detach().float().contiguous(), g, b, eps, act=act, tail=0,
                                                         save=need)
        ctx.rng, ctx.ffn, ctx.act = rng, ffn, act
        ctx.caches = (cache1, cache2, cache_d, cache_u)
        ctx.inp_is_x = inp is x
        if need:
            ctx.save_for_backward(h, z, mean, rstd, g, s, u_ad, u, w1, w2, w_down, w_up)
        return out

    @staticmethod
    def backward(ctx, dout):
        h, z, mean, rstd, g, s, u_ad, u, w1, w2, w_down, w_up = ctx.saved_tensors
        cache1, cache2, cache_d, cache_u = ctx.caches
        dout = dout.contiguous()
        dg = db = None
        if ctx.needs_input_grad[13] or ctx.needs_input_grad[14]:
            dg, db = torch.empty_like(g), torch.empty_like(g)
        dz = ops.layernorm_bwd(dout, z, mean, rstd, g, dgamma=dg, dbeta=db)
        _, wut = cache_u.get(w_up, need_t=True)
        _, wdt = cache_d.get(w_down, need_t=True)
        if ctx.act == "gelu":
            ds = ops.gemm(dz, wut, epilogue=ops.EPI_DGELU, aux=u_ad)
        else:
            ds = ops.gemm(dz, wut, epilogue=ops.EPI_DRELU, aux=s)
        dwd = ops.wgrad(ds, h) if ctx.needs_input_grad[9] else None
        dbd = ops.colsum(ds) if ctx.needs_input_grad[10] else None
        dwu = dbu = None
        if ctx.needs_input_grad[11] or ctx.needs_input_grad[12]:
            full = ops.wgrad(dz, ops.s_ext(s))
            dwu, dbu = full[:, :s.shape[1]], full[:, s.shape[1]]
        dx = None
        if ctx.needs_input_grad[0]:
            dhm = ops.gemm(ds, wdt, residual=dz, dropout=ctx.rng, dropout_after=True)
            fold = dz if ctx.inp_is_x else None
            _, w1t = cache1.get(w1, need_t=True)
            if ctx.ffn:
                _, w2t = cache2.get(w2, need_t=True)
                du = ops.gemm(dhm, w2t, epilogue=ops.EPI_DGELU, aux=u)
                dx = ops.gemm(du, w1t, residual=fold)
            else:
                dx = ops.gemm(dhm, w1t, residual=fold)
        dinp = dz if (ctx.needs_input_grad[1] and not ctx.inp_is_x) else None
        return (dx, dinp, None, None, None, None, None, None, None, dwd, dbd, dwu, dbu, dg, db, None, None, None, None)


def houlsby_postln_block(x, inp, p, dense, intermediate, adapter, ln):
    if intermediate is None:
        w1, b1, c1, w2, b2, c2 = dense.weight, dense.bias, dense._cache, None, None, None
    else:
        w1, b1, c1 = intermediate.weight, intermediate.bias, intermediate._cache
        w2, b2, c2 = dense.weight, dense.bias, dense._cache
    return HoulsbyPostLNBlockFunction.apply(x, inp, p, w1, b1, c1, w2, b2, c2, adapter.fc_down.weight, adapter.fc_down.bias,
                                            adapter.fc_up.weight, adapter.fc_up.bias, ln.weight, ln.bias, ln.eps,
                                            adapter.act, adapter.fc_down._cache, adapter.fc_up._cache)


class IdEmbeddingFunction(torch.autograd.Function):

    @staticmethod
    def forward(ctx, ids, weight, padding_idx):
        emb, hist = ops.id_embed_fwd(weight.detach(), ids)
        ctx.save_for_backward(ids)
        ctx.weight, ctx.padding_idx = weight, padding_idx
        return emb, hist

    @staticmethod
    def backward(ctx, d_emb, d_hist):
        (ids,) = ctx.saved_tensors
        w = ctx.weight
        if d_emb is None and d_hist is None:
            return None, None, None
        if w.grad is None:
            w.grad = torch.zeros_like(w)
        ref = d_emb if d_emb is not None else d_hist
        B, S1 = ids.shape[0], ids.shape[1]
        if d_emb is None:
            d_emb = torch.zeros((B, S1, 2, w.shape[1]), dtype=ref.dtype, device=ref.device)
        ops.id_embed_bwd(ids, d_emb.contiguous(), None if d_hist is None else d_hist.contiguous(), w.grad,
                         padding_idx=ctx.padding_idx, accumulate=True)
        return None, None, None


def id_embedding(ids, weight, padding_idx=0):
    return IdEmbeddingFunction.apply(ids, weight, padding_idx)
```

### adapter4rec_b200/lib.py

```python
import ctypes
import os
from ctypes import POINTER, Structure, c_char_p, c_float, c_int32, c_int64, c_size_t, c_void_p

HERE = os.path.dirname(os.path.abspath(__file__))
LIB_PATH = os.path.join(HERE, "libadapter4rec_sm100.so")

A4R_OK, A4R_EINVAL, A4R_ECUDA, A4R_EARCH, A4R_EWORKSPACE = 0, -1, -2, -3, -4
EPI_LINEAR, EPI_GELU, EPI_RELU, EPI_DGELU, EPI_DRELU = 0, 1, 2, 3, 4


class GemmArgs(Structure):
    _fields_ = [
        ("A", c_void_p), ("lda", c_int64), ("B", c_void_p), ("ldb", c_int64),
        ("A2", c_void_p), ("lda2", c_int64), ("B2", c_void_p), ("ldb2", c_int64), ("K2", c_int64),
        ("C", c_void_p), ("ldc", c_int64), ("aux", c_void_p), ("ldaux", c_int64),
        ("residual", c_void_p), ("ldr", c_int64), ("residual2", c_void_p), ("ldr2", c_int64),
        ("bias", c_void_p), ("M", c_int64), ("N", c_int64), ("K", c_int64),
        ("alpha", c_float), ("epilogue", c_int32), ("out_f32", c_int32), ("block_n", c_int32),
        ("dropout_p", c_float), ("dropout_seed", ctypes.c_uint64), ("dropout_offset", ctypes.c_uint64),
        ("dropout_after_residual", c_int32),
    ]


class AttnArgs(Structure):
    _fields_ = [
        ("qkv", c_void_p), ("out", c_void_p), ("dout", c_void_p), ("mask", c_void_p),
        ("ld_qkv", c_int64), ("ld_out", c_int64), ("mask_ld", c_int64),
        ("N", c_int64), ("L", c_int64), ("heads", c_int64), ("head_dim", c_int64),
        ("mask_dtype", c_int32), ("causal", c_int32), ("scale", c_float), ("mask_neg", c_float),
        ("lse", c_void_p), ("ctx", c_void_p),
        ("dropout_p", c_float), ("dropout_seed", ctypes.c_uint64), ("dropout_offset", ctypes.c_uint64),
        ("cu_seqlens", c_void_p),
    ]


class EmbedArgs(Structure):
    _fields_ = [
        ("ids", c_void_p), ("ld_ids", c_int64), ("word_emb", c_void_p), ("pos_emb", c_void_p),
        ("type_emb", c_void_p), ("prompt", c_void_p), ("gamma", c_void_p), ("beta", c_void_p),
        ("out", c_void_p), ("z_out", c_void_p), ("mean_out", c_void_p), ("rstd_out", c_void_p),
        ("N", c_int64), ("L", c_int64), ("H", c_int64), ("pos_offset", c_int64),
        ("roberta_pad_id", c_int64), ("n_prompt", c_int64), ("eps", c_float),
    ]


class BceArgs(Structure):
    _fields_ = [
        ("prec", c_void_p), ("emb", c_void_p), ("log_mask", c_void_p), ("pos_score", c_void_p),
        ("neg_score", c_void_p), ("loss", c_void_p), ("count", c_void_p),
        ("B", c_int64), ("S", c_int64), ("D", c_int64), ("cpc", c_int32),
    ]


class AdapterArgs(Structure):
    _fields_ = [
        ("h", c_void_p), ("ldh", c_int64), ("input", c_void_p), ("ldi", c_int64),
        ("w_down", c_void_p), ("b_down", c_void_p), ("w_up", c_void_p), ("b_up", c_void_p),
        ("gamma", c_void_p), ("beta", c_void_p), ("out", c_void_p), ("z_out", c_void_p),
        ("mean", c_void_p), ("rstd", c_void_p), ("s_out", c_void_p), ("u_out", c_void_p),
        ("M", c_int64), ("H", c_int64), ("r", c_int64), ("act", c_int32), ("tail", c_int32), ("eps", c_float),
        ("lds", c_int64), ("impl", c_int32),
    ]


class InbatchCeArgs(Structure):
    _fields_ = [
        ("prec", c_void_p), ("cand", c_void_p), ("ld_cand", c_int64), ("item_ids", c_void_p), ("log_mask", c_void_p),
        ("cand_bias", c_void_p), ("lse", c_void_p), ("loss", c_void_p), ("count", c_void_p),
        ("B", c_int64), ("S", c_int64), ("D", c_int64), ("masked_logit", c_float),
    ]


PROTOTYPES = {
    "a4r_version": (c_int32, []),
    "a4r_last_error_string": (c_char_p, []),
    "a4r_device_check": (c_int32, []),
    "a4r_launch_count": (c_int64, []),
    "a4r_gemm_bf16_tn": (c_int32, [POINTER(GemmArgs), c_void_p]),
    "a4r_attn_small_fwd": (c_int32, [POINTER(AttnArgs), c_void_p]),
    "a4r_attn_small_bwd": (c_int32, [POINTER(AttnArgs), c_void_p]),
    "a4r_attn_mid_fwd": (c_int32, [POINTER(AttnArgs), c_void_p]),
    "a4r_attn_mid_bwd": (c_int32, [POINTER(AttnArgs), c_void_p]),
    "a4r_layernorm_fwd": (c_int32, [c_void_p, c_void_p, c_int64, c_void_p, c_void_p, c_float, c_void_p, c_void_p,
                                    c_void_p, c_void_p, c_int64, c_int64, c_void_p]),
    "a4r_layernorm_bwd_workspace_bytes": (c_size_t, [c_int64]),
    "a4r_layernorm_bwd": (c_int32, [c_void_p, c_void_p, c_void_p, c_void_p, c_void_p, c_void_p, c_void_p, c_void_p,
                                    c_int32, c_void_p, c_size_t, c_int64, c_int64, c_void_p, c_float, ctypes.c_uint64,
                                    ctypes.c_uint64, c_void_p]),
    "a4r_layernorm_bwd_add": (c_int32, [c_void_p, c_void_p, c_void_p, c_void_p, c_void_p, c_void_p, c_void_p, c_int64, c_int64,
                                        c_void_p]),
    "a4r_adapter_ln_supported": (c_int32, [c_int64, c_int64]),
    "a4r_adapter_ln_fwd": (c_int32, [POINTER(AdapterArgs), c_void_p]),
    "a4r_embed_ln_fwd": (c_int32, [POINTER(EmbedArgs), c_void_p]),
    "a4r_act_bwd": (c_int32, [c_void_p, c_void_p, c_void_p, c_int64, c_int32, c_void_p]),
    "a4r_act_fwd": (c_int32, [c_void_p, c_void_p, c_int64, c_int32, c_void_p]),
    "a4r_scatter_add_rows": (c_int32, [c_void_p, c_int64, c_void_p, c_void_p, c_int64, c_int64, c_int64, c_int64, c_void_p]),
    "a4r_cast_transpose_f32_bf16": (c_int32, [c_void_p, c_int64, c_void_p, c_void_p, c_int64, c_int64, c_void_p]),
    "a4r_dropout": (c_int32, [c_void_p, c_void_p, c_void_p, c_int64, c_float, ctypes.c_uint64, ctypes.c_uint64, c_void_p]),
    "a4r_colsum_workspace_bytes": (c_size_t, [c_int64]),
    "a4r_colsum": (c_int32, [c_void_p, c_int64, c_int64, c_int64, c_void_p, c_int32, c_void_p, c_size_t, c_void_p]),
    "a4r_wgrad_workspace_bytes": (c_size_t, [c_int64, c_int64, c_int64]),
    "a4r_wgrad_bf16": (c_int32, [c_void_p, c_int64, c_void_p, c_int64, c_void_p, c_int64, c_int64, c_int64, c_int64,
                                 c_float, c_int32, c_void_p, c_size_t, c_void_p]),
    "a4r_wgrad_tc_workspace_bytes": (c_size_t, [c_int64, c_int64, c_int64]),
    "a4r_wgrad_tc_bf16": (c_int32, [c_void_p, c_int64, c_void_p, c_int64, c_void_p, c_int64, c_int64, c_int64, c_int64,
                                    c_float, c_int32, c_void_p, c_size_t, c_void_p]),
    "a4r_bce_workspace_bytes": (c_size_t, []),
    "a4r_bce_loss_fwd": (c_int32, [POINTER(BceArgs), c_void_p, c_size_t, c_void_p]),
    "a4r_bce_loss_bwd": (c_int32, [POINTER(BceArgs), c_void_p, c_void_p, c_void_p, c_void_p]),
    "a4r_inbatch_ce_workspace_bytes": (c_size_t, [c_int64, c_int64]),
    "a4r_inbatch_ce_fwd": (c_int32, [POINTER(InbatchCeArgs), c_void_p, c_size_t, c_void_p]),
    "a4r_inbatch_ce_bwd": (c_int32, [POINTER(InbatchCeArgs), c_void_p, c_void_p, c_void_p, c_int64, c_void_p]),
    "a4r_adam_step": (c_int32, [c_void_p, c_void_p, c_void_p, c_void_p, c_int64, c_float, c_float, c_float, c_float,
                                c_float, c_int64, c_float, c_void_p]),
    "a4r_adam_step_dev": (c_int32, [c_void_p, c_void_p, c_void_p, c_void_p, c_int64, c_float, c_float, c_float, c_float,
                                    c_float, c_void_p, c_float, c_void_p]),
    "a4r_patchify": (c_int32, [c_void_p, c_void_p, c_int64, c_int64, c_int64, c_int64, c_void_p]),
    "a4r_vit_assemble": (c_int32, [c_void_p, c_void_p, c_void_p, c_void_p, c_void_p, c_int64, c_int64, c_int64, c_int64,
                                   c_void_p]),
    "a4r_gather_rows": (c_int32, [c_void_p, c_void_p, c_void_p, c_int64, c_int64, c_void_p]),
    "a4r_sample_train_batch": (c_int32, [c_void_p, c_void_p, c_void_p, c_void_p, c_void_p, c_void_p, c_void_p, c_int64,
                                         c_int64, c_int64, c_int64, ctypes.c_uint64, ctypes.c_uint64, c_void_p]),
    "a4r_id_embed_fwd": (c_int32, [c_void_p, c_int64, c_int64, c_void_p, c_int64, c_int64, c_void_p, c_void_p, c_void_p]),
    "a4r_id_embed_bwd": (c_int32, [c_void_p, c_void_p, c_void_p, c_void_p, c_void_p, c_int64, c_int64, c_int64, c_int64,
                                   c_int64, c_int32, c_void_p]),
    "a4r_score_topk_partials": (c_int32, [c_int64, c_int64]),
    "a4r_score_topk": (c_int32, [c_void_p, c_int64, c_void_p, c_int64, c_int64, c_int64, c_int64, c_int64, c_void_p,
                                 c_int64, c_int32, c_void_p, c_void_p, c_void_p]),
    "a4r_topk_merge": (c_int32, [c_void_p, c_void_p, c_int32, c_int64, c_int32, c_void_p, c_void_p, c_void_p, c_void_p,
                                 c_void_p, c_void_p]),
}

_lib = None


def get_lib():
    global _lib
    if _lib is None:
        if not os.path.exists(LIB_PATH):
            raise RuntimeError(
                "adapter4rec_b200: %s is missing — build it with __graft_entry__.build() "
                "(there is no CPU or PyTorch fallback for this path)" % LIB_PATH)
        lib = ctypes.CDLL(LIB_PATH)
        for name, (restype, argtypes) in PROTOTYPES.items():
            fn = getattr(lib, name)
            fn.restype = restype
            fn.argtypes = argtypes
        _lib = lib
    return _lib


def check(rc, what):
    if rc != A4R_OK:
        msg = get_lib().a4r_last_error_string()
        raise RuntimeError("%s failed (code %d): %s" % (what, rc, msg.decode() if msg else ""))


def launch_count():
    return int(get_lib().a4r_launch_count())
```

### adapter4rec_b200/model/bert.py

```python
import torch
import torch.nn as nn

from .. import functional as Fn
from .. import ops
from .layers import BF16, Embedding, LayerNorm, Linear, LoRALinear, to_2d_bf16


class TextConfigLite:

    def __init__(self, hf_config=None, **kw):
        src = {} if hf_config is None else {k: getattr(hf_config, k) for k in dir(hf_config) if not k.startswith("_")
                                            and isinstance(getattr(hf_config, k, None), (int, float, str, bool, type(None)))}
        src.update(kw)
        self.vocab_size = src.get("vocab_size", 30522)
        self.hidden_size = src.get("hidden_size", 768)
        self.num_hidden_layers = src.get("num_hidden_layers", 12)
        self.num_attention_heads = src.get("num_attention_heads", 12)
        self.intermediate_size = src.get("intermediate_size", 3072)
        self.max_position_embeddings = src.get("max_position_embeddings", 512)
        self.type_vocab_size = src.get("type_vocab_size", 2)
        self.layer_norm_eps = src.get("layer_norm_eps", 1e-12)
        self.pad_token_id = src.get("pad_token_id", 0)
        self.model_type = src.get("model_type", "bert")
        self.hidden_dropout_prob = src.get("hidden_dropout_prob", 0.1)
        self.attention_probs_dropout_prob = src.get("attention_probs_dropout_prob", 0.1)
        self.initializer_range = src.get("initializer_range", 0.02)


class BertEmbeddings(nn.Module):
    def __init__(self, config):
        super().__init__()
        self.config = config
        self.word_embeddings = Embedding(config.vocab_size, config.hidden_size, padding_idx=config.pad_token_id)
        self.position_embeddings = Embedding(config.max_position_embeddings, config.hidden_size)
        self.token_type_embeddings = Embedding(config.type_vocab_size, config.hidden_size)
        self.LayerNorm = LayerNorm(config.hidden_size, eps=config.layer_norm_eps)
        self.dropout = nn.Dropout(config.hidden_dropout_prob)
        self._typ_cache = Fn.WeightCache()

    def forward(self, input_ids):
        N, L = input_ids.shape
        we = self.word_embeddings
        prompt = None
        if hasattr(we, "learned_embedding"):
            prompt, table = we.learned_embedding, we.wte.table_bf16()
            assert we.n_tokens <= L
        else:
            table = we.table_bf16()
        roberta_pad = self.config.pad_token_id if self.config.model_type == "roberta" else -1
        typ = self._typ_cache.get(self.token_type_embeddings.weight)[0][0]
        tables = (table, self.position_embeddings.table_bf16(), typ)
        g, b = self.LayerNorm.weight.detach().float(), self.LayerNorm.bias.detach().float()
        wmaster = we.wte.weight if hasattr(we, "learned_embedding") else we.weight
        masters = [wmaster, self.position_embeddings.weight, self.token_type_embeddings.weight, self.LayerNorm.weight,
                   self.LayerNorm.bias]
        masters = [m if m.requires_grad else None for m in masters]
        x = Fn.EmbedLNFunction.apply(input_ids, L, tables, g, b, self.LayerNorm.eps, roberta_pad, prompt,
                                     int(self.config.pad_token_id), *masters)
        if self.training and self.dropout.p > 0:
            x = Fn.dropout_add(x, None, self.dropout.p)
        return x


class BertSelfAttention(nn.Module):
    def __init__(self, config):
        super().__init__()
        self.num_attention_heads = config.num_attention_heads
        self.attention_head_size = config.hidden_size // config.num_attention_heads
        self.all_head_size = config.hidden_size
        self.query = Linear(config.hidden_size, config.hidden_size)
        self.key = Linear(config.hidden_size, config.hidden_size)
        self.value = Linear(config.hidden_size, config.hidden_size)
        self.dropout = nn.Dropout(config.attention_probs_dropout_prob)
        self._qkv_cache = {}

    def forward(self, x2d, attention_mask, N, L, packed=None, want_skip=False):
        params = []
        for m in (self.query, self.key, self.value):
            params += [m.weight, m.bias, getattr(m, "lora_A", None), getattr(m, "lora_B", None)]
        skip = x2d
        if want_skip and x2d.requires_grad:
            qkv, skip = Fn.QKVFunction.apply(x2d, self._qkv_cache, *params, "skip")
        else:
            qkv = Fn.QKVFunction.apply(x2d, self._qkv_cache, *params)
        if packed is not None:
            ctx = Fn.attention(qkv, packed.token_mask, N, L, self.num_attention_heads, self.attention_head_size,
                               causal=False, mask_neg=ops.F32_MIN, dropout_p=self.dropout.p if self.training else 0.0,
                               cu_seqlens=packed.cu_seqlens)
        else:
            ctx = Fn.attention(qkv, attention_mask, N, L, self.num_attention_heads, self.attention_head_size,
                               causal=False, mask_neg=ops.F32_MIN, dropout_p=self.dropout.p if self.training else 0.0)
        return (ctx, skip) if want_skip else ctx


class BertSelfOutput(nn.Module):

    def __init__(self, config, in_features=None):
        super().__init__()
        self.dense = Linear(in_features or config.hidden_size, config.hidden_size)
        self.LayerNorm = LayerNorm(config.hidden_size, eps=config.layer_norm_eps)
        self.dropout = nn.Dropout(config.hidden_dropout_prob)

    def forward(self, hidden_states, input_tensor):
        shape = input_tensor.shape
        p = self.dropout.p if self.training else 0.0
        d = self.dense
        if not (d.weight.requires_grad or d.bias.requires_grad):
            out = Fn.PostLNBlockFunction.apply(to_2d_bf16(hidden_states), to_2d_bf16(input_tensor), self.LayerNorm.weight,
                                               self.LayerNorm.bias, self.LayerNorm.eps, p, d.weight, d.bias, d._cache,
                                               None, None, None)
            return out.view(shape)
        if p > 0:
            z = Fn.dropout_add(d(to_2d_bf16(hidden_states)), to_2d_bf16(input_tensor).contiguous(), p)
        else:
            z = d(to_2d_bf16(hidden_states), residual=to_2d_bf16(input_tensor))
        return self.LayerNorm(z).view(shape)


class BertOutput(BertSelfOutput):
    def __init__(self, config):
        super().__init__(config, in_features=config.intermediate_size)


class BertAttention(nn.Module):
    def __init__(self, config):
        super().__init__()
        self.self = BertSelfAttention(config)
        self.output = BertSelfOutput(config)

    def forward(self, x2d, attention_mask, N, L, packed=None):
        ctx, skip = self.self(x2d, attention_mask, N, L, packed, want_skip=True)
        return self.output(ctx, skip)


class BertIntermediate(nn.Module):
    def __init__(self, config):
        super().__init__()
        self.dense = Linear(config.hidden_size, config.intermediate_size)

    def forward(self, x):
        return self.dense(x, act="gelu")


class BertLayer(nn.Module):
    def __init__(self, config):
        super().__init__()
        self.attention = BertAttention(config)
        self.intermediate = BertIntermediate(config)
        self.output = BertOutput(config)

    def forward(self, x2d, attention_mask, N, L, cls_only=False, packed=None):
        if cls_only:
            H = x2d.shape[1]
            ctx, skip = self.attention.self(x2d, attention_mask, N, L, packed, want_skip=True)
            if packed is not None:
                y = self.attention.output(Fn.gather_rows(ctx, packed.cls_rows), Fn.gather_rows(skip, packed.cls_rows))
            else:
                y = self.attention.output(ctx.view(N, L, H)[:, 0], skip.view(N, L, H)[:, 0])
        else:
            y = self.attention(x2d, attention_mask, N, L, packed)
        out = self.output
        wi = self.intermediate.dense
        inner = out.self_output if hasattr(out, "self_output") else out
        wf = getattr(inner, "dense", None)
        frozen = wf is not None and not (wi.weight.requires_grad or wi.bias.requires_grad or
                                         wf.weight.requires_grad or wf.bias.requires_grad)
        if frozen and type(out) is BertOutput:
            p = out.dropout.p if self.training else 0.0
            return Fn.PostLNBlockFunction.apply(y, y, out.LayerNorm.weight, out.LayerNorm.bias, out.LayerNorm.eps, p,
                                                wi.weight, wi.bias, wi._cache, wf.weight, wf.bias, wf._cache)
        if frozen and hasattr(out, "forward_block"):
            fused = out.forward_block(y, y, wi)
            if fused is not None:
                return to_2d_bf16(fused)
        if frozen and hasattr(out, "forward_from_dense"):
            h = Fn.FFNFunction.apply(y, wi.weight, wi.bias, wf.weight, wf.bias, None, wi._cache, wf._cache)
            return to_2d_bf16(out.forward_from_dense(h, y))
        return out(self.intermediate(y), y)


class PackedTokens:

    def __init__(self, attention_mask):
        m = attention_mask != 0
        keep = m | (~m.any(dim=1, keepdim=True))
        flat = keep.reshape(-1)
        self.token_rows = flat.nonzero().squeeze(1)
        lens = keep.sum(dim=1)
        cu = torch.zeros(m.shape[0] + 1, dtype=torch.int32, device=m.device)
        cu[1:] = torch.cumsum(lens, 0)
        self.cu_seqlens = cu
        self.cls_rows = cu[:-1].long()
        self.token_mask = m.reshape(-1)[self.token_rows].float().contiguous()
        self.num_tokens = int(self.token_rows.numel())


class BertEncoder(nn.Module):
    def __init__(self, config):
        super().__init__()
        self.layer = nn.ModuleList([BertLayer(config) for _ in range(config.num_hidden_layers)])


class BertPooler(nn.Module):

    def __init__(self, config):
        super().__init__()
        self.dense = Linear(config.hidden_size, config.hidden_size)


class BertModel(nn.Module):

    def __init__(self, config, add_pooling_layer=True):
        super().__init__()
        self.config = config if isinstance(config, TextConfigLite) else TextConfigLite(config)
        self.embeddings = BertEmbeddings(self.config)
        self.encoder = BertEncoder(self.config)
        self.pooler = BertPooler(self.config) if add_pooling_layer else None
        self.apply(self._init_weights)

    def _init_weights(self, module):
        std = self.config.initializer_range
        if isinstance(module, (Linear, Embedding)):
            nn.init.normal_(module.weight, mean=0.0, std=std)
            if getattr(module, "bias", None) is not None:
                nn.init.zeros_(module.bias)
        elif isinstance(module, LayerNorm):
            nn.init.ones_(module.weight)
            nn.init.zeros_(module.bias)

    def get_input_embeddings(self):
        return self.embeddings.word_embeddings

    def set_input_embeddings(self, value):
        self.embeddings.word_embeddings = value

    supports_cls_only = True

    def forward(self, input_ids=None, attention_mask=None, cls_only=False, output_hidden_states=None, **unused):
        N, L = input_ids.shape
        if output_hidden_states is None:
            output_hidden_states = bool(getattr(self.config, "output_hidden_states", False))
        x = self.embeddings(input_ids)
        all_hidden = [x.view(N, L, -1)] if output_hidden_states else None
        last = len(self.encoder.layer) - 1
        packed = None
        if (getattr(self, "unpad", False) and cls_only and not output_hidden_states and attention_mask is not None
                and L <= 32 and not x.requires_grad):
            packed = PackedTokens(attention_mask)
            x = Fn.gather_rows(x, packed.token_rows)
        for i, layer in enumerate(self.encoder.layer):
            x = layer(x, attention_mask, N, L, cls_only=cls_only and i == last and not output_hidden_states, packed=packed)
            if output_hidden_states:
                all_hidden.append(x.view(N, L, -1))
        if output_hidden_states:
            return (x.view(N, L, -1), None, tuple(all_hidden))
        return (x.view(N, 1 if cls_only else L, -1),)


class RobertaModel(BertModel):
    def __init__(self, config, add_pooling_layer=True):
        cfg = config if isinstance(config, TextConfigLite) else TextConfigLite(config)
        cfg.model_type = "roberta"
        super().__init__(cfg, add_pooling_layer)
```

### adapter4rec_b200/ops.py

```python
import ctypes

import torch

from . import lib as _l
from .lib import EPI_DGELU, EPI_DRELU, EPI_GELU, EPI_LINEAR, EPI_RELU

BF16 = torch.bfloat16
F32_MIN = -3.4028234663852886e38


def _stream():
    return ctypes.c_void_p(torch.cuda.current_stream().cuda_stream)


def _p(t):
    return None if t is None else ctypes.c_void_p(t.data_ptr())


def _rows2d(t, name):
    if t.dim() != 2 or t.stride(1) != 1:
        raise ValueError("%s must be 2-D with unit column stride, got shape %s stride %s" % (name, tuple(t.shape), t.stride()))
    return t.stride(0) if t.shape[0] > 1 else max(t.stride(0), t.shape[1])


_workspaces = {}


def workspace(nbytes, device):
    key = (device.index, torch.cuda.current_stream(device).cuda_stream)
    ws = _workspaces.get(key)
    if ws is None or ws.numel() < nbytes:
        ws = torch.empty(max(int(nbytes), 1 << 20), dtype=torch.uint8, device=device)
        _workspaces[key] = ws
    return ws


_gemm_profile = None


def gemm_profile_start():
    global _gemm_profile
    _gemm_profile = []


def gemm_profile_stop(by_shape=False):
    global _gemm_profile
    prof, _gemm_profile = _gemm_profile, None
    torch.cuda.synchronize()
    flops = sum(p[0] for p in prof)
    times = [p[1].elapsed_time(p[2]) for p in prof]
    ms = sum(times)
    if not by_shape:
        return flops, ms, len(prof)
    groups = {}
    for p, t in zip(prof, times):
        g = groups.setdefault(p[3], [0.0, 0.0, 0])
        g[0] += p[0]
        g[1] += t
        g[2] += 1
    return flops, ms, len(prof), groups


def gemm(a, b, bias=None, epilogue=EPI_LINEAR, residual=None, residual2=None, aux=None, a2=None, b2=None,
         alpha=1.0, out=None, out_dtype=BF16, block_n=0, dropout=None, dropout_after=False):
    assert a.dtype == BF16 and b.dtype == BF16, "gemm operands must be bf16"
    M, K = a.shape
    N, Kb = b.shape
    assert K == Kb, "gemm: K mismatch %d vs %d" % (K, Kb)
    if out is None:
        out = torch.empty((M, N), dtype=out_dtype, device=a.device)
    g = _l.GemmArgs()
    g.A, g.lda = _p(a), _rows2d(a, "a")
    g.B, g.ldb = _p(b), _rows2d(b, "b")
    if a2 is not None:
        assert a2.dtype == BF16 and b2.dtype == BF16 and a2.shape[0] == M and b2.shape[0] == N and a2.shape[1] == b2.shape[1]
        g.A2, g.lda2, g.B2, g.ldb2, g.K2 = _p(a2), _rows2d(a2, "a2"), _p(b2), _rows2d(b2, "b2"), a2.shape[1]
    g.C, g.ldc = _p(out), _rows2d(out, "out")
    if aux is not None:
        assert aux.dtype == BF16 and tuple(aux.shape) == (M, N)
        g.aux, g.ldaux = _p(aux), _rows2d(aux, "aux")
    if residual is not None:
        assert residual.dtype == BF16 and tuple(residual.shape) == (M, N)
        g.residual, g.ldr = _p(residual), _rows2d(residual, "residual")
    if residual2 is not None:
        assert residual2.dtype == BF16 and tuple(residual2.shape) == (M, N)
        g.residual2, g.ldr2 = _p(residual2), _rows2d(residual2, "residual2")
    if bias is not None:
        assert bias.dtype == torch.float32 and bias.numel() == N and bias.is_contiguous()
        g.bias = _p(bias)
    g.M, g.N, g.K = M, N, K
    if dropout is not None:
        assert out.is_contiguous(), "epilogue dropout indexes the logical [M, N] output"
        g.dropout_p, g.dropout_seed, g.dropout_offset = float(dropout[0]), int(dropout[1]), int(dropout[2])
        g.dropout_after_residual = int(bool(dropout_after))
    g.alpha, g.epilogue, g.out_f32, g.block_n = float(alpha), int(epilogue), int(out.dtype == torch.float32), int(block_n)
    assert out.dtype in (BF16, torch.float32)
    if _gemm_profile is not None:
        e0, e1 = torch.cuda.Event(enable_timing=True), torch.cuda.Event(enable_timing=True)
        e0.record()
        _l.check(_l.get_lib().a4r_gemm_bf16_tn(ctypes.byref(g), _stream()), "a4r_gemm_bf16_tn")
        e1.record()
        k2 = a2.shape[1] if a2 is not None else 0
        _gemm_profile.append((2.0 * M * N * (K + k2), e0, e1, (M, N, K + k2, int(epilogue))))
        return out
    _l.check(_l.get_lib().a4r_gemm_bf16_tn(ctypes.byref(g), _stream()), "a4r_gemm_bf16_tn")
    return out


def dropout(x, res, p, seed, offset):
    assert x.dtype == BF16 and x.is_contiguous() and (res is None or (res.dtype == BF16 and res.is_contiguous() and res.shape == x.shape))
    out = torch.empty_like(x)
    _l.check(_l.get_lib().a4r_dropout(_p(x), _p(res), _p(out), x.numel(), float(p), int(seed), int(offset), _stream()),
             "a4r_dropout")
    return out


def _attn_args(qkv, N, L, heads, head_dim, mask, causal, mask_neg, dropout=None, scale=None, cu_seqlens=None):
    a = _l.AttnArgs()
    if cu_seqlens is not None:
        assert cu_seqlens.dtype == torch.int32 and cu_seqlens.is_contiguous() and cu_seqlens.numel() == N + 1 and L <= 32
        a.cu_seqlens = _p(cu_seqlens)
        if mask is not None:
            assert mask.dim() == 1 and mask.numel() == qkv.shape[0] and mask.is_contiguous()
            a.mask, a.mask_ld = _p(mask), 0
            a.mask_dtype = {torch.int64: 1, torch.float32: 2}[mask.dtype]
    if dropout is not None:
        a.dropout_p, a.dropout_seed, a.dropout_offset = float(dropout[0]), int(dropout[1]), int(dropout[2])
    a.qkv, a.ld_qkv = _p(qkv), _rows2d(qkv, "qkv")
    a.N, a.L, a.heads, a.head_dim = N, L, heads, head_dim
    if mask is None:
        a.mask_dtype = 0
    elif cu_seqlens is None:
        assert mask.dim() == 2 and mask.shape[0] == N and mask.shape[1] >= L and mask.stride(1) == 1
        a.mask, a.mask_ld = _p(mask), mask.stride(0)
        a.mask_dtype = {torch.int64: 1, torch.float32: 2}[mask.dtype]
    a.causal, a.scale, a.mask_neg = int(causal), (float(head_dim) ** -0.5 if scale is None else float(scale)), float(mask_neg)
    return a


def _attn_kernel(L, head_dim, causal, direction):
    lib = _l.get_lib()
    if L <= 32:
        return (lib.a4r_attn_small_fwd if direction == "fwd" else lib.a4r_attn_small_bwd), "a4r_attn_small_" + direction
    if L <= 256 and head_dim == 64 and not causal:
        return (lib.a4r_attn_mid_fwd if direction == "fwd" else lib.a4r_attn_mid_bwd), "a4r_attn_mid_" + direction
    raise RuntimeError("attention: unsupported shape L=%d head_dim=%d causal=%s (no fallback exists)" % (L, head_dim, causal))


def attn_small_fwd(qkv, N, L, heads, head_dim, mask=None, causal=False, mask_neg=F32_MIN, want_lse=False, dropout=None,
                   scale=None, cu_seqlens=None):
    assert qkv.dtype == BF16 and (cu_seqlens is not None or qkv.shape[0] == N * L)
    out = torch.empty((qkv.shape[0], heads * head_dim), dtype=BF16, device=qkv.device)
    a = _attn_args(qkv, N, L, heads, head_dim, mask, causal, mask_neg, dropout, scale, cu_seqlens)
    a.out, a.ld_out = _p(out), out.stride(0)
    lse = None
    if want_lse and L > 32:
        lse = torch.empty((N * L, heads), dtype=torch.float32, device=qkv.device)
        a.lse = _p(lse)
    fn, name = _attn_kernel(L, head_dim, causal, "fwd")
    _l.check(fn(ctypes.byref(a), _stream()), name)
    return (out, lse) if want_lse else out


def attn_small_bwd(qkv, dctx, N, L, heads, head_dim, mask=None, causal=False, mask_neg=F32_MIN, lse=None, ctx=None,
                   dropout=None, scale=None, cu_seqlens=None):
    assert qkv.dtype == BF16 and dctx.dtype == BF16 and dctx.shape[0] == qkv.shape[0]
    assert cu_seqlens is not None or qkv.shape[0] == N * L
    dqkv = torch.empty((qkv.shape[0], 3 * heads * head_dim), dtype=BF16, device=qkv.device)
    a = _attn_args(qkv, N, L, heads, head_dim, mask, causal, mask_neg, dropout, scale, cu_seqlens)
    assert _rows2d(qkv, "qkv") == dqkv.stride(0), "attention bwd expects a contiguous qkv"
    a.out, a.dout, a.ld_out = _p(dqkv), _p(dctx), _rows2d(dctx, "dctx")
    if L > 32:
        assert lse is not None and ctx is not None and ctx.is_contiguous() and dctx.is_contiguous()
        a.lse, a.ctx = _p(lse), _p(ctx)
    fn, name = _attn_kernel(L, head_dim, causal, "bwd")
    _l.check(fn(ctypes.byref(a), _stream()), name)
    return dqkv


def layernorm_fwd(x, gamma, beta, eps, res=None, want_z=False, want_stats=True):
    assert x.dtype == BF16 and x.is_contiguous() and x.dim() == 2
    M, H = x.shape
    y = torch.empty_like(x)
    z = torch.empty_like(x) if want_z else None
    mean = torch.empty(M, dtype=torch.float32, device=x.device) if want_stats else None
    rstd = torch.empty(M, dtype=torch.float32, device=x.device) if want_stats else None
    res_rows = 0
    if res is not None:
        assert res.dtype == BF16 and res.is_contiguous() and res.shape[-1] == H
        res_rows = res.numel() // H
    _l.check(_l.get_lib().a4r_layernorm_fwd(_p(x), _p(res), res_rows, _p(gamma), _p(beta), float(eps), _p(y), _p(z),
                                            _p(mean), _p(rstd), M, H, _stream()), "a4r_layernorm_fwd")
    return y, z, mean, rstd


def layernorm_bwd(dy, z, mean, rstd, gamma, dgamma=None, dbeta=None, accumulate=False, masked=None):
    assert dy.dtype == BF16 and z.dtype == BF16 and dy.is_contiguous() and z.is_contiguous()
    M, H = z.shape
    dz = torch.empty_like(z)
    dzm = torch.empty_like(z) if masked is not None else None
    mp, mseed, moff = masked if masked is not None else (0.0, 0, 0)
    ws, wsb = None, 0
    if dgamma is not None:
        wsb = _l.get_lib().a4r_layernorm_bwd_workspace_bytes(H)
        ws = workspace(wsb, z.device)
    _l.check(_l.get_lib().a4r_layernorm_bwd(_p(dy), _p(z), _p(mean), _p(rstd), _p(gamma), _p(dz), _p(dgamma), _p(dbeta),
                                            int(accumulate), _p(ws), wsb, M, H, _p(dzm), float(mp), int(mseed), int(moff),
                                            _stream()), "a4r_layernorm_bwd")
    return (dz, dzm) if masked is not None else dz


def layernorm_bwd_add(dy, z, mean, rstd, gamma, dskip):
    assert dy.dtype == BF16 and z.dtype == BF16 and dskip.dtype == BF16
    assert dy.is_contiguous() and z.is_contiguous() and dskip.is_contiguous() and dskip.shape == z.shape
    M, H = z.shape
    dz = torch.empty_like(z)
    _l.check(_l.get_lib().a4r_layernorm_bwd_add(_p(dy), _p(z), _p(mean), _p(rstd), _p(gamma), _p(dskip), _p(dz), M, H,
                                                _stream()), "a4r_layernorm_bwd_add")
    return dz


def embed_ln_fwd(ids, L, word_emb, pos_emb, type_emb, gamma, beta, eps, pos_offset=0, roberta_pad_id=-1, prompt=None,
                 want_z=False):
    assert ids.dtype == torch.int64 and ids.dim() == 2 and ids.stride(1) == 1
    N, H = ids.shape[0], word_emb.shape[1]
    out = torch.empty((N * L, H), dtype=BF16, device=ids.device)
    z = torch.empty_like(out) if want_z else None
    mean = torch.empty(N * L, dtype=torch.float32, device=ids.device) if want_z else None
    rstd = torch.empty(N * L, dtype=torch.float32, device=ids.device) if want_z else None
    a = _l.EmbedArgs()
    a.ids, a.ld_ids = _p(ids), ids.stride(0)
    a.word_emb, a.pos_emb, a.type_emb, a.prompt = _p(word_emb), _p(pos_emb), _p(type_emb), _p(prompt)
    a.gamma, a.beta, a.out, a.z_out, a.mean_out, a.rstd_out = _p(gamma), _p(beta), _p(out), _p(z), _p(mean), _p(rstd)
    a.N, a.L, a.H, a.pos_offset, a.roberta_pad_id = N, L, H, pos_offset, roberta_pad_id
    a.n_prompt = 0 if prompt is None else prompt.shape[0]
    a.eps = float(eps)
    _l.check(_l.get_lib().a4r_embed_ln_fwd(ctypes.byref(a), _stream()), "a4r_embed_ln_fwd")
    return out, z, mean, rstd


def scatter_add_rows(src, idx, num_rows, skip_idx=-1):
    assert src.dtype == BF16 and src.dim() == 2 and src.stride(1) == 1 and idx.dtype == torch.int64
    idx = idx.contiguous().view(-1)
    assert idx.numel() == src.shape[0]
    out = torch.zeros((num_rows, src.shape[1]), dtype=torch.float32, device=src.device)
    _l.check(_l.get_lib().a4r_scatter_add_rows(_p(src), src.stride(0), _p(idx), _p(out), src.shape[0], src.shape[1],
                                               int(num_rows), int(skip_idx), _stream()), "a4r_scatter_add_rows")
    return out


ACT_KINDS = {"gelu": 0, "relu": 1, "leaky_relu": 2, "gelu_new": 3}


def act_bwd(dy, u, kind):
    assert dy.dtype == BF16 and u.dtype == BF16 and dy.is_contiguous() and u.is_contiguous() and dy.shape == u.shape
    out = torch.empty_like(dy)
    _l.check(_l.get_lib().a4r_act_bwd(_p(dy), _p(u), _p(out), dy.numel(), ACT_KINDS[kind], _stream()), "a4r_act_bwd")
    return out


def cast_transpose(w, want=True, want_t=False):
    assert w.dtype == torch.float32 and w.dim() == 2 and w.stride(1) == 1
    rows, cols = w.shape
    out = torch.empty((rows, cols), dtype=BF16, device=w.device) if want else None
    out_t = torch.empty((cols, rows), dtype=BF16, device=w.device) if want_t else None
    _l.check(_l.get_lib().a4r_cast_transpose_f32_bf16(_p(w), w.stride(0), _p(out), _p(out_t), rows, cols, _stream()),
             "a4r_cast_transpose_f32_bf16")
    return out, out_t


def act_fwd(u, kind):
    assert u.dtype == BF16 and u.is_contiguous()
    out = torch.empty_like(u)
    _l.check(_l.get_lib().a4r_act_fwd(_p(u), _p(out), u.numel(), ACT_KINDS[kind], _stream()), "a4r_act_fwd")
    return out


def colsum(x, width=None, out=None, accumulate=False):
    assert x.dtype == BF16 and x.dim() == 2
    M = x.shape[0]
    width = x.shape[1] if width is None else width
    if out is None and width == x.shape[1] and width <= 128 and x.is_contiguous() and M >= 4096:
        f = 16
        while f > 1 and M % f:
            f //= 2
        if f > 1:
            return colsum(x.view(M // f, f * width)).view(f, width).sum(0)
    if out is None:
        out = torch.empty(width, dtype=torch.float32, device=x.device)
        accumulate = False
    wsb = _l.get_lib().a4r_colsum_workspace_bytes(width)
    ws = workspace(wsb, x.device)
    _l.check(_l.get_lib().a4r_colsum(_p(x), _rows2d(x, "x"), M, width, _p(out), int(accumulate), _p(ws), wsb, _stream()),
             "a4r_colsum")
    return out


def wgrad_mma_sync(a, b, alpha=1.0, out=None, accumulate=False, n=None, k=None):
    assert a.dtype == BF16 and b.dtype == BF16 and a.shape[0] == b.shape[0]
    M = a.shape[0]
    N = a.shape[1] if n is None else n
    K = b.shape[1] if k is None else k
    if out is None:
        out = torch.empty((N, K), dtype=torch.float32, device=a.device)
        accumulate = False
    assert out.dtype == torch.float32 and tuple(out.shape) == (N, K) and out.stride(1) == 1
    wsb = _l.get_lib().a4r_wgrad_workspace_bytes(M, N, K)
    ws = workspace(wsb, a.device)
    _l.check(_l.get_lib().a4r_wgrad_bf16(_p(a), _rows2d(a, "a"), _p(b), _rows2d(b, "b"), _p(out), out.stride(0), M, N, K,
                                         float(alpha), int(accumulate), _p(ws), wsb, _stream()), "a4r_wgrad_bf16")
    return out


def wgrad_tc(a, b, alpha=1.0, out=None, accumulate=False, n=None, k=None):
    assert a.dtype == BF16 and b.dtype == BF16 and a.shape[0] == b.shape[0]
    M = a.shape[0]
    N = a.shape[1] if n is None else n
    K = b.shape[1] if k is None else k
    if out is None:
        out = torch.empty((N, K), dtype=torch.float32, device=a.device)
        accumulate = False
    assert out.dtype == torch.float32 and tuple(out.shape) == (N, K) and out.stride(1) == 1
    wsb = _l.get_lib().a4r_wgrad_tc_workspace_bytes(M, N, K)
    ws = workspace(wsb, a.device)
    _l.check(_l.get_lib().a4r_wgrad_tc_bf16(_p(a), _rows2d(a, "a"), _p(b), _rows2d(b, "b"), _p(out), out.stride(0), M, N, K,
                                            float(alpha), int(accumulate), _p(ws), wsb, _stream()), "a4r_wgrad_tc_bf16")
    return out


wgrad = wgrad_tc


def _bce_args(prec, emb, log_mask, pos, neg, loss, count, cpc):
    B, S, D = prec.shape
    assert prec.dtype == BF16 and emb.dtype == BF16 and prec.is_contiguous() and emb.is_contiguous()
    assert emb.numel() == B * (S + 1) * 2 * D
    a = _l.BceArgs()
    a.prec, a.emb, a.log_mask = _p(prec), _p(emb), _p(log_mask)
    a.pos_score, a.neg_score, a.loss, a.count = _p(pos), _p(neg), _p(loss), _p(count)
    a.B, a.S, a.D, a.cpc = B, S, D, int(cpc)
    return a


def bce_loss_fwd(prec, emb, log_mask, cpc=False):
    B, S, _ = prec.shape
    dev = prec.device
    pos = torch.empty((B, S), dtype=torch.float32, device=dev)
    neg = torch.empty((B, S), dtype=torch.float32, device=dev)
    loss = torch.empty(1, dtype=torch.float32, device=dev)
    count = torch.empty(1, dtype=torch.float32, device=dev)
    if log_mask is not None:
        assert log_mask.dtype == torch.float32 and log_mask.is_contiguous() and tuple(log_mask.shape) == (B, S)
    a = _bce_args(prec, emb, log_mask, pos, neg, loss, count, cpc)
    wsb = _l.get_lib().a4r_bce_workspace_bytes()
    ws = workspace(wsb, dev)
    _l.check(_l.get_lib().a4r_bce_loss_fwd(ctypes.byref(a), _p(ws), wsb, _stream()), "a4r_bce_loss_fwd")
    return loss, count, pos, neg


def bce_loss_bwd(prec, emb, log_mask, pos, neg, count, grad_out=None, cpc=False):
    d_prec = torch.empty_like(prec)
    d_emb = torch.empty_like(emb)
    loss = torch.empty(1, dtype=torch.float32, device=prec.device)
    a = _bce_args(prec, emb, log_mask, pos, neg, loss, count, cpc)
    if grad_out is not None:
        assert grad_out.dtype == torch.float32 and grad_out.numel() == 1
    _l.check(_l.get_lib().a4r_bce_loss_bwd(ctypes.byref(a), _p(grad_out), _p(d_prec), _p(d_emb), _stream()),
             "a4r_bce_loss_bwd")
    return d_prec, d_emb


def adapter_ln_supported(H, r):
    return bool(_l.get_lib().a4r_adapter_ln_supported(int(H), int(r)))


def adapter_ln_fwd(h, inp, w_down, b_down, w_up, b_up, gamma=None, beta=None, eps=0.0, act="relu", tail=0, save=False,
                   impl=0):
    assert h.dtype == BF16 and h.dim() == 2 and w_down.dtype == BF16 and w_up.dtype == BF16
    assert w_down.is_contiguous() and w_up.is_contiguous()
    M, H = h.shape
    r = w_down.shape[0]
    assert tuple(w_down.shape) == (r, H) and tuple(w_up.shape) == (H, r)
    for t in (b_down, b_up) + ((gamma, beta) if tail == 0 else ()):
        assert t.dtype == torch.float32 and t.is_contiguous()
    dev = h.device
    out = torch.empty((M, H), dtype=BF16, device=dev)
    z = mean = rstd = s = u = None
    if save:
        s = torch.empty((M, r + 16), dtype=BF16, device=dev)[:, :r]
        if act == "gelu":
            u = torch.empty((M, r), dtype=BF16, device=dev)
        if tail == 0:
            z = torch.empty((M, H), dtype=BF16, device=dev)
            mean = torch.empty(M, dtype=torch.float32, device=dev)
            rstd = torch.empty(M, dtype=torch.float32, device=dev)
    a = _l.AdapterArgs()
    a.h, a.ldh = _p(h), _rows2d(h, "h")
    if inp is not None:
        assert inp.dtype == BF16 and tuple(inp.shape) == (M, H)
        a.input, a.ldi = _p(inp), _rows2d(inp, "input")
    a.w_down, a.b_down, a.w_up, a.b_up = _p(w_down), _p(b_down), _p(w_up), _p(b_up)
    a.gamma, a.beta, a.out, a.z_out, a.mean, a.rstd, a.s_out, a.u_out = (_p(gamma), _p(beta), _p(out), _p(z), _p(mean),
                                                                         _p(rstd), _p(s), _p(u))
    a.M, a.H, a.r, a.act, a.tail, a.eps = M, H, r, {"relu": 0, "gelu": 1}[act], int(tail), float(eps)
    a.lds = 0 if s is None else s.stride(0)
    a.impl = int(impl)
    _l.check(_l.get_lib().a4r_adapter_ln_fwd(ctypes.byref(a), _stream()), "a4r_adapter_ln_fwd")
    return out, z, mean, rstd, s, u


def s_ext(s):
    M, r = s.shape
    assert s.stride(0) == r + 16 and s.storage_offset() == 0
    return s.as_strided((M, r + 8), (r + 16, 1))


MASKED_LOGIT = -1e4


def _inbatch_args(prec, emb, item_ids, log_mask, cand_bias, lse, loss, count):
    B, S, D = prec.shape
    assert prec.dtype == BF16 and emb.dtype == BF16 and prec.is_contiguous() and emb.is_contiguous()
    assert emb.numel() == B * (S + 1) * 2 * D, "emb must be Model.forward's encoder output [B, S+1, 2, D]"
    assert item_ids.dtype == torch.int64 and item_ids.is_contiguous() and tuple(item_ids.shape) == (B, S + 1)
    assert log_mask.dtype == torch.float32 and log_mask.is_contiguous() and tuple(log_mask.shape) == (B, S)
    if cand_bias is not None:
        assert cand_bias.dtype == torch.float32 and cand_bias.is_contiguous() and cand_bias.numel() == B * (S + 1)
    a = _l.InbatchCeArgs()
    a.prec, a.cand, a.ld_cand = _p(prec), _p(emb), 2 * D
    a.item_ids, a.log_mask, a.cand_bias = _p(item_ids), _p(log_mask), _p(cand_bias)
    a.lse, a.loss, a.count = _p(lse), _p(loss), _p(count)
    a.B, a.S, a.D, a.masked_logit = B, S, D, MASKED_LOGIT
    return a


def inbatch_ce_fwd(prec, emb, item_ids, log_mask, cand_bias=None):
    B, S, _ = prec.shape
    dev = prec.device
    lse = torch.empty(B * S, dtype=torch.float32, device=dev)
    loss = torch.empty(1, dtype=torch.float32, device=dev)
    count = torch.empty(1, dtype=torch.float32, device=dev)
    a = _inbatch_args(prec, emb, item_ids, log_mask, cand_bias, lse, loss, count)
    wsb = _l.get_lib().a4r_inbatch_ce_workspace_bytes(B, S)
    ws = workspace(wsb, dev)
    _l.check(_l.get_lib().a4r_inbatch_ce_fwd(ctypes.byref(a), _p(ws), wsb, _stream()), "a4r_inbatch_ce_fwd")
    return loss, count, lse


def inbatch_ce_bwd(prec, emb, item_ids, log_mask, lse, count, cand_bias=None, grad_out=None):
    d_prec = torch.empty_like(prec)
    d_emb = torch.zeros_like(emb)
    loss = torch.empty(1, dtype=torch.float32, device=prec.device)
    a = _inbatch_args(prec, emb, item_ids, log_mask, cand_bias, lse, loss, count)
    if grad_out is not None:
        assert grad_out.dtype == torch.float32 and grad_out.numel() == 1
    _l.check(_l.get_lib().a4r_inbatch_ce_bwd(ctypes.byref(a), _p(grad_out), _p(d_prec), _p(d_emb), 2 * prec.shape[2],
                                             _stream()), "a4r_inbatch_ce_bwd")
    return d_prec, d_emb


def adam_step(p, g, m, v, lr, beta1, beta2, eps, weight_decay, step, grad_scale=1.0):
    for t in (p, g, m, v):
        assert t.dtype == torch.float32 and t.is_contiguous() and t.numel() == p.numel()
    _l.check(_l.get_lib().a4r_adam_step(_p(p), _p(g), _p(m), _p(v), p.numel(), float(lr), float(beta1), float(beta2),
                                        float(eps), float(weight_decay), int(step), float(grad_scale), _stream()),
             "a4r_adam_step")


def adam_step_dev(p, g, m, v, lr, beta1, beta2, eps, weight_decay, bias_corr, grad_scale=1.0):
    for t in (p, g, m, v):
        assert t.dtype == torch.float32 and t.is_contiguous() and t.numel() == p.numel()
    assert bias_corr.dtype == torch.float32 and bias_corr.numel() == 2 and bias_corr.is_cuda
    _l.check(_l.get_lib().a4r_adam_step_dev(_p(p), _p(g), _p(m), _p(v), p.numel(), float(lr), float(beta1), float(beta2),
                                            float(eps), float(weight_decay), _p(bias_corr), float(grad_scale), _stream()),
             "a4r_adam_step_dev")


def adam_bias_corrections(beta1, beta2, step):
    import math
    import struct
    b1, b2 = (struct.unpack("f", struct.pack("f", float(b)))[0] for b in (beta1, beta2))
    return 1.0 - math.pow(b1, int(step)), math.sqrt(1.0 - math.pow(b2, int(step)))


def gather_rows(table, ids):
    assert table.dtype == BF16 and table.is_contiguous() and ids.dtype == torch.int64
    ids_c = ids.contiguous()
    out = torch.empty(tuple(ids.shape) + (table.shape[1],), dtype=BF16, device=table.device)
    _l.check(_l.get_lib().a4r_gather_rows(_p(table), _p(ids_c), _p(out), ids_c.numel(), table.shape[1], _stream()),
             "a4r_gather_rows")
    return out


def sample_train_batch(seqs, item_content, item_num, seed, offset, neg_in=None):
    assert seqs.dtype == torch.int64 and seqs.is_contiguous() and seqs.dim() == 2
    B, S1 = seqs.shape
    dev = seqs.device
    if item_content is None:
        W, out = 0, None
    else:
        assert item_content.dtype == torch.int64 and item_content.is_contiguous() and item_content.dim() == 2
        W = item_content.shape[1]
        out = torch.empty((B, S1, 2, W), dtype=torch.int64, device=dev)
    log_mask = torch.empty((B, S1 - 1), dtype=torch.float32, device=dev)
    neg = torch.empty((B, S1), dtype=torch.int64, device=dev)
    fail = torch.zeros(1, dtype=torch.int32, device=dev)
    if neg_in is not None:
        assert neg_in.dtype == torch.int64 and neg_in.is_contiguous() and neg_in.shape == seqs.shape
    _l.check(_l.get_lib().a4r_sample_train_batch(_p(seqs), _p(item_content), _p(neg_in), _p(out), _p(log_mask), _p(neg),
                                                 _p(fail), B, S1, W, int(item_num), int(seed) & (2 ** 64 - 1),
                                                 int(offset) & (2 ** 64 - 1), _stream()), "a4r_sample_train_batch")
    return out, log_mask, neg, fail


def id_embed_fwd(table, ids, want_hist=True):
    assert table.dtype == torch.float32 and table.dim() == 2 and table.is_contiguous()
    assert ids.dtype == torch.int64 and ids.dim() == 3 and ids.shape[2] == 2 and ids.is_contiguous()
    B, S1, _ = ids.shape
    V, D = table.shape
    emb = torch.empty((B, S1, 2, D), dtype=BF16, device=table.device)
    hist = torch.empty((B, S1 - 1, D), dtype=BF16, device=table.device) if want_hist else None
    _l.check(_l.get_lib().a4r_id_embed_fwd(_p(table), V, D, _p(ids), B, S1, _p(emb), _p(hist), _stream()),
             "a4r_id_embed_fwd")
    return emb, hist


def id_embed_bwd(ids, d_emb, d_hist, grad, padding_idx=0, accumulate=True):
    assert ids.dtype == torch.int64 and ids.dim() == 3 and ids.shape[2] == 2 and ids.is_contiguous()
    B, S1, _ = ids.shape
    V, D = grad.shape
    assert grad.dtype == torch.float32 and grad.is_contiguous()
    assert d_emb.dtype == BF16 and d_emb.is_contiguous() and d_emb.numel() == B * S1 * 2 * D
    if d_hist is not None:
        assert d_hist.dtype == BF16 and d_hist.is_contiguous() and d_hist.numel() == B * (S1 - 1) * D
    sorted_ids, order = torch.sort(ids.view(-1), stable=True)
    _l.check(_l.get_lib().a4r_id_embed_bwd(_p(sorted_ids), _p(order), _p(d_emb), _p(d_hist), _p(grad), V, D, B, S1,
                                           int(padding_idx), int(bool(accumulate)), _stream()), "a4r_id_embed_bwd")
    return grad


def score_topk(users, items, id_base=0, history=None, k=10):
    assert users.dtype == BF16 and items.dtype == BF16 and users.shape[1] == items.shape[1]
    U, d = users.shape
    I = items.shape[0]
    P = _l.get_lib().a4r_score_topk_partials(U, I)
    sc = torch.empty((P, U, k), dtype=torch.float32, device=users.device)
    ids = torch.empty((P, U, k), dtype=torch.int32, device=users.device)
    hl = 0
    if history is not None:
        assert history.dtype == torch.int32 and history.is_contiguous() and history.shape[0] == U
        hl = history.shape[1]
    _l.check(_l.get_lib().a4r_score_topk(_p(users), _rows2d(users, "users"), _p(items), _rows2d(items, "items"), U, I, d,
                                         int(id_base), _p(history), hl, int(k), _p(sc), _p(ids), _stream()),
             "a4r_score_topk")
    return sc, ids


def topk_merge(scores, ids, target=None):
    P, U, k = scores.shape
    assert scores.dtype == torch.float32 and ids.dtype == torch.int32 and scores.is_contiguous() and ids.is_contiguous()
    osc = torch.empty((U, k), dtype=torch.float32, device=scores.device)
    oid = torch.empty((U, k), dtype=torch.int32, device=scores.device)
    hit = ndcg = None
    if target is not None:
        assert target.dtype == torch.int32 and target.numel() == U and target.is_contiguous()
        hit = torch.empty(U, dtype=torch.float32, device=scores.device)
        ndcg = torch.empty(U, dtype=torch.float32, device=scores.device)
    _l.check(_l.get_lib().a4r_topk_merge(_p(scores), _p(ids), P, U, k, _p(osc), _p(oid), _p(target), _p(hit), _p(ndcg),
                                         _stream()), "a4r_topk_merge")
    return osc, oid, hit, ndcg


def patchify(images, patch_size):
    assert images.dtype == torch.float32 and images.is_contiguous() and images.dim() == 4 and images.shape[2] == images.shape[3]
    N, C, R, _ = images.shape
    P = (R // patch_size) ** 2
    out = torch.empty((N * P, C * patch_size * patch_size), dtype=BF16, device=images.device)
    _l.check(_l.get_lib().a4r_patchify(_p(images), _p(out), N, C, R, patch_size, _stream()), "a4r_patchify")
    return out


def vit_assemble(patch_emb, cls, pos, prompt, N, P):
    H = patch_emb.shape[1]
    T = 0 if prompt is None else prompt.shape[0]
    for t in (patch_emb, cls, pos) + ((prompt,) if prompt is not None else ()):
        assert t.dtype == BF16 and t.is_contiguous()
    out = torch.empty((N * (1 + P + T), H), dtype=BF16, device=patch_emb.device)
    _l.check(_l.get_lib().a4r_vit_assemble(_p(patch_emb), _p(cls), _p(pos), _p(prompt), _p(out), N, P, T, H, _stream()),
             "a4r_vit_assemble")
    return out
```

### include/adapter4rec.h

```cpp
#ifndef ADAPTER4REC_H_
#define ADAPTER4REC_H_

#include <stddef.h>
#include <stdint.h>

#ifdef __cplusplus
extern "C" {
#endif

#define A4R_OK 0
#define A4R_EINVAL (-1)
#define A4R_ECUDA (-2)
#define A4R_EARCH (-3)
#define A4R_EWORKSPACE (-4)

typedef void* a4r_stream_t;

#define A4R_API __attribute__((visibility("default")))

A4R_API int a4r_version(void);
A4R_API const char* a4r_last_error_string(void);
A4R_API int a4r_device_check(void);
A4R_API int64_t a4r_launch_count(void);

enum {
  A4R_EPI_LINEAR = 0,
  A4R_EPI_GELU = 1,
  A4R_EPI_RELU = 2,
  A4R_EPI_DGELU = 3,
  A4R_EPI_DRELU = 4
};

typedef struct a4r_gemm_args {
  const void* A;
  int64_t lda;
  const void* B;
  int64_t ldb;
  const void* A2;
  int64_t lda2;
  const void* B2;
  int64_t ldb2;
  int64_t K2;
  void* C;
  int64_t ldc;
  void* aux;
  int64_t ldaux;
  const void* residual;
  int64_t ldr;
  const void* residual2;
  int64_t ldr2;
  const float* bias;
  int64_t M, N, K;
  float alpha;
  int32_t epilogue;
  int32_t out_f32;
  int32_t block_n;
  float dropout_p;
  uint64_t dropout_seed;
  uint64_t dropout_offset;
  int32_t dropout_after_residual;
} a4r_gemm_args;

A4R_API int a4r_gemm_bf16_tn(const a4r_gemm_args* args, a4r_stream_t stream);

typedef struct a4r_attn_args {
  const void* qkv;
  void* out;
  const void* dout;
  const void* mask;
  int64_t ld_qkv, ld_out, mask_ld;
  int64_t N, L, heads, head_dim;
  int32_t mask_dtype;
  int32_t causal;
  float scale;
  float mask_neg;
  float* lse;
  const void* ctx;
  float dropout_p;
  uint64_t dropout_seed;
  uint64_t dropout_offset;
  const int32_t* cu_seqlens;
} a4r_attn_args;

A4R_API int a4r_attn_small_fwd(const a4r_attn_args* args, a4r_stream_t stream);
A4R_API int a4r_attn_small_bwd(const a4r_attn_args* args, a4r_stream_t stream);

A4R_API int a4r_attn_mid_fwd(const a4r_attn_args* args, a4r_stream_t stream);
A4R_API int a4r_attn_mid_bwd(const a4r_attn_args* args, a4r_stream_t stream);

A4R_API int a4r_layernorm_fwd(const void* x, const void* res, int64_t res_rows, const float* gamma, const float* beta,
                      float eps, void* y, void* z_out, float* mean, float* rstd, int64_t M, int64_t H,
                      a4r_stream_t stream);
A4R_API size_t a4r_layernorm_bwd_workspace_bytes(int64_t H);
A4R_API int a4r_layernorm_bwd(const void* dy, const void* z, const float* mean, const float* rstd, const float* gamma,
                      void* dz, float* dgamma, float* dbeta, int32_t accumulate, void* workspace,
                      size_t workspace_bytes, int64_t M, int64_t H, void* dz_masked, float dropout_p,
                      uint64_t dropout_seed, uint64_t dropout_offset, a4r_stream_t stream);
A4R_API int a4r_layernorm_bwd_add(const void* dy, const void* z, const float* mean, const float* rstd, const float* gamma,
                          const void* dskip, void* dz, int64_t M, int64_t H, a4r_stream_t stream);

typedef struct a4r_adapter_args {
  const void* h;
  int64_t ldh;
  const void* input;
  int64_t ldi;
  const void* w_down;
  const float* b_down;
  const void* w_up;
  const float* b_up;
  const float* gamma;
  const float* beta;
  void* out;
  void* z_out;
  float* mean;
  float* rstd;
  void* s_out;
  void* u_out;
  int64_t M, H, r;
  int32_t act;
  int32_t tail;
  float eps;
  int64_t lds;
  int32_t impl;
} a4r_adapter_args;
A4R_API int a4r_adapter_ln_supported(int64_t H, int64_t r);
A4R_API int a4r_adapter_ln_fwd(const a4r_adapter_args* args, a4r_stream_t stream);

typedef struct a4r_embed_args {
  const int64_t* ids;
  int64_t ld_ids;
  const void* word_emb;
  const void* pos_emb;
  const void* type_emb;
  const void* prompt;
  const float* gamma;
  const float* beta;
  void* out;
  void* z_out;
  float* mean_out;
  float* rstd_out;
  int64_t N, L, H;
  int64_t pos_offset;
  int64_t roberta_pad_id;
  int64_t n_prompt;
  float eps;
} a4r_embed_args;
A4R_API int a4r_embed_ln_fwd(const a4r_embed_args* args, a4r_stream_t stream);

A4R_API int a4r_patchify(const float* images, void* out, int64_t N, int64_t C, int64_t R, int64_t ps, a4r_stream_t stream);
A4R_API int a4r_vit_assemble(const void* patch_emb, const void* cls, const void* pos, const void* prompt, void* out,
                             int64_t N, int64_t P, int64_t T, int64_t H, a4r_stream_t stream);

A4R_API int a4r_scatter_add_rows(const void* src, int64_t ld, const int64_t* idx, float* dst, int64_t R, int64_t H,
                                 int64_t V, int64_t skip_idx, a4r_stream_t stream);

A4R_API int a4r_act_bwd(const void* dy, const void* u, void* out, int64_t n, int32_t kind, a4r_stream_t stream);
A4R_API int a4r_act_fwd(const void* u, void* out, int64_t n, int32_t kind, a4r_stream_t stream);

A4R_API int a4r_cast_transpose_f32_bf16(const float* src, int64_t ld_src, void* dst, void* dst_t, int64_t rows, int64_t cols,
                                        a4r_stream_t stream);

A4R_API int a4r_dropout(const void* x, const void* res, void* out, int64_t n, float p, uint64_t seed, uint64_t offset,
                        a4r_stream_t stream);
#define A4R_SEED_INDIRECT (1ull << 63)

A4R_API size_t a4r_colsum_workspace_bytes(int64_t width);
A4R_API int a4r_colsum(const void* x, int64_t ld, int64_t M, int64_t width, float* out, int32_t accumulate,
               void* workspace, size_t workspace_bytes, a4r_stream_t stream);

A4R_API size_t a4r_wgrad_workspace_bytes(int64_t M, int64_t N, int64_t K);
A4R_API int a4r_wgrad_bf16(const void* A, int64_t lda, const void* B, int64_t ldb, float* dW, int64_t ldw, int64_t M,
                   int64_t N, int64_t K, float alpha, int32_t accumulate, void* workspace, size_t workspace_bytes,
                   a4r_stream_t stream);

A4R_API size_t a4r_wgrad_tc_workspace_bytes(int64_t M, int64_t N, int64_t K);
A4R_API int a4r_wgrad_tc_bf16(const void* A, int64_t lda, const void* B, int64_t ldb, float* dW, int64_t ldw, int64_t M,
                              int64_t N, int64_t K, float alpha, int32_t accumulate, void* workspace,
                              size_t workspace_bytes, a4r_stream_t stream);

typedef struct a4r_bce_args {
  const void* prec;
  const void* emb;
  const float* log_mask;
  float* pos_score;
  float* neg_score;
  float* loss;
  float* count;
  int64_t B, S, D;
  int32_t cpc;
} a4r_bce_args;
A4R_API size_t a4r_bce_workspace_bytes(void);
A4R_API int a4r_bce_loss_fwd(const a4r_bce_args* args, void* workspace, size_t workspace_bytes, a4r_stream_t stream);
A4R_API int a4r_bce_loss_bwd(const a4r_bce_args* args, const float* grad_out, void* d_prec, void* d_emb,
                     a4r_stream_t stream);

typedef struct a4r_inbatch_ce_args {
  const void* prec;
  const void* cand;
  int64_t ld_cand;
  const int64_t* item_ids;
  const float* log_mask;
  const float* cand_bias;
  float* lse;
  float* loss;
  float* count;
  int64_t B, S, D;
  float masked_logit;
} a4r_inbatch_ce_args;
A4R_API size_t a4r_inbatch_ce_workspace_bytes(int64_t B, int64_t S);
A4R_API int a4r_inbatch_ce_fwd(const a4r_inbatch_ce_args* args, void* workspace, size_t workspace_bytes, a4r_stream_t stream);
A4R_API int a4r_inbatch_ce_bwd(const a4r_inbatch_ce_args* args, const float* grad_out, void* d_prec, void* d_cand,
                               int64_t ld_dcand, a4r_stream_t stream);

A4R_API int a4r_adam_step(float* p, const float* g, float* m, float* v, int64_t n, float lr, float beta1, float beta2,
                  float eps, float weight_decay, int64_t step, float grad_scale, a4r_stream_t stream);
A4R_API int a4r_adam_step_dev(float* p, const float* g, float* m, float* v, int64_t n, float lr, float beta1, float beta2,
                              float eps, float weight_decay, const float* bias_corr, float grad_scale, a4r_stream_t stream);

A4R_API int a4r_gather_rows(const void* table, const int64_t* ids, void* out, int64_t rows, int64_t D,
                            a4r_stream_t stream);

A4R_API int a4r_sample_train_batch(const int64_t* seqs, const int64_t* item_content, const int64_t* neg_in, int64_t* out,
                                   float* log_mask, int64_t* neg_out, int32_t* fail_flag, int64_t B, int64_t S1, int64_t W,
                                   int64_t item_num, uint64_t seed, uint64_t offset, a4r_stream_t stream);

A4R_API int a4r_id_embed_fwd(const float* table, int64_t V, int64_t D, const int64_t* ids, int64_t B, int64_t S1,
                             void* emb, void* hist, a4r_stream_t stream);
A4R_API int a4r_id_embed_bwd(const int64_t* sorted_ids, const int64_t* order, const void* d_emb, const void* d_hist,
                             float* grad, int64_t V, int64_t D, int64_t B, int64_t S1, int64_t padding_idx,
                             int32_t accumulate, a4r_stream_t stream);

A4R_API int a4r_score_topk_partials(int64_t U, int64_t I);
A4R_API int a4r_score_topk(const void* users, int64_t ld_users, const void* items, int64_t ld_items, int64_t U, int64_t I,
                           int64_t d, int64_t id_base, const int32_t* history, int64_t hist_len, int32_t k,
                           float* out_scores, int32_t* out_ids, a4r_stream_t stream);

A4R_API int a4r_topk_merge(const float* in_scores, const int32_t* in_ids, int32_t P, int64_t U, int32_t k,
                           float* out_scores, int32_t* out_ids, const int32_t* target, float* hit, float* ndcg,
                           a4r_stream_t stream);

#ifdef __cplusplus
}
#endif
#endif
```

Before: 1947.

## Add CLS-query-only attention mode and double-buffer the short-sequence backward kernel

Adds a cls_query_only mode to the short-sequence attention kernel so the last BERT layer, which only needs the [CLS] output, computes and stores a single query row per head and reads a single dO row in backward. The backward kernel is restructured to prefetch the next unit's Q/K/V/dO into a second smem buffer with cp.async groups. It also computes dQ, dK and dV sequentially to reduce live registers, reuses the V tile for P, changes warps per CTA, and computes dropout keep bits ahead of the wait. This adds smem per warp and more complex buffer handling in exchange for less wasted work and better latency hiding.

```diff
diff --git a/adapter4rec_b200/csrc/attention_mid.cu b/adapter4rec_b200/csrc/attention_mid.cu
--- a/adapter4rec_b200/csrc/attention_mid.cu
+++ b/adapter4rec_b200/csrc/attention_mid.cu
@@ -376,6 +376,7 @@
   A4R_CHECK_ARG(a->head_dim == DH, "attention_mid: head_dim must be 64");
   A4R_CHECK_ARG(a->causal == 0, "attention_mid: causal masking is not supported (use the short-sequence kernel)");
   A4R_CHECK_ARG(a->dropout_p == 0.0f, "attention_mid: probability dropout is not implemented (ViT uses p = 0)");
+  A4R_CHECK_ARG(a->cls_query_only == 0, "attention_mid: the [CLS]-query mode is short-sequence only");
   A4R_CHECK_ARG(a->heads >= 1 && a->N >= 0, "attention_mid: bad heads/N");
   A4R_CHECK_ARG(a->ld_qkv >= 3 * a->heads * DH && a->ld_qkv % 8 == 0 && a->ld_out >= a->heads * DH && a->ld_out % 8 == 0,
                 "attention_mid: bad leading dimensions");
diff --git a/adapter4rec_b200/csrc/attention_small.cu b/adapter4rec_b200/csrc/attention_small.cu
--- a/adapter4rec_b200/csrc/attention_small.cu
+++ b/adapter4rec_b200/csrc/attention_small.cu
@@ -4,7 +4,6 @@
 namespace {
 
 constexpr int LP = 32;
-constexpr int WARPS_PER_CTA = 4;
 
 struct AttnParams {
   const __nv_bfloat16* qkv;
@@ -20,12 +19,13 @@
   uint32_t drop_thr16;
   float drop_scale;
   uint64_t drop_seed, drop_offset;
+  int cls_query;
 };
 
-A4R_DEVICE void prob_dropout(float (&s)[2][4][4], const AttnParams& p, int n, int h, int lane) {
+A4R_DEVICE uint32_t prob_keep_bits(uint64_t seed, const AttnParams& p, int n, int h, int lane) {
   const int g = lane >> 2, t = lane & 3;
   const uint64_t base = p.drop_offset + (static_cast<uint64_t>(n) * p.heads + h) * (32 * 8);
-  const uint64_t seed = rng_seed(p.drop_seed);
+  uint32_t keep = 0;
 #pragma unroll
   for (int mt = 0; mt < 2; ++mt)
 #pragma unroll
@@ -37,12 +37,22 @@
 #pragma unroll
         for (int q = 0; q < 2; ++q)
 #pragma unroll
-          for (int e = 0; e < 2; ++e) {
-            float& x = s[mt][np * 2 + q][hh * 2 + e];
-            x = rng_keep(r, q * 2 + e, p.drop_thr16) ? x * p.drop_scale : 0.0f;
-          }
-      }
-    }
+          for (int e = 0; e < 2; ++e)
+            if (rng_keep(r, q * 2 + e, p.drop_thr16)) keep |= 1u << ((mt * 4 + np * 2 + q) * 4 + hh * 2 + e);
+      }
+    }
+  return keep;
+}
+A4R_DEVICE void prob_dropout(float (&s)[2][4][4], uint32_t keep, float drop_scale) {
+#pragma unroll
+  for (int mt = 0; mt < 2; ++mt)
+#pragma unroll
+    for (int nt = 0; nt < 4; ++nt)
+#pragma unroll
+      for (int c = 0; c < 4; ++c) {
+        float& x = s[mt][nt][c];
+        x = ((keep >> ((mt * 4 + nt) * 4 + c)) & 1u) ? x * drop_scale : 0.0f;
+      }
 }
 
 template <int COLS>
@@ -98,7 +108,11 @@
                  : "memory");
   }
 }
-A4R_DEVICE void cp_async_wait_all() { asm volatile("cp.async.wait_all;" ::: "memory"); }
+A4R_DEVICE void cp_async_commit() { asm volatile("cp.async.commit_group;" ::: "memory"); }
+template <int PENDING>
+A4R_DEVICE void cp_async_wait() {
+  asm volatile("cp.async.wait_group %0;" ::"n"(PENDING) : "memory");
+}
 template <int DH>
 A4R_DEVICE void store_tile(const uint8_t* tile, __nv_bfloat16* g, int64_t ld, int L, int lane) {
   constexpr int CH = DH / 8;
@@ -139,10 +153,27 @@
   }
   return s;
 }
-A4R_DEVICE bool key_valid(const AttnParams& p, const SeqSpan& sq, int j) {
-  if (p.mask_dtype == 1) return reinterpret_cast<const int64_t*>(p.mask)[sq.mask0 + j] != 0;
-  if (p.mask_dtype == 2) return reinterpret_cast<const float*>(p.mask)[sq.mask0 + j] != 0.0f;
-  return true;
+struct Unit {
+  int n, h;
+  SeqSpan sq;
+  uint64_t mask_raw;
+};
+A4R_DEVICE Unit unit_at(const AttnParams& p, int64_t w, int lane) {
+  Unit u;
+  u.n = static_cast<int>(w / p.heads), u.h = static_cast<int>(w % p.heads);
+  u.sq = seq_span(p, u.n);
+  u.mask_raw = 0;
+  if (lane < u.sq.L) {
+    if (p.mask_dtype == 1) u.mask_raw = static_cast<uint64_t>(reinterpret_cast<const int64_t*>(p.mask)[u.sq.mask0 + lane]);
+    if (p.mask_dtype == 2) u.mask_raw = __float_as_uint(reinterpret_cast<const float*>(p.mask)[u.sq.mask0 + lane]);
+  }
+  return u;
+}
+A4R_DEVICE uint32_t unit_keymask(const AttnParams& p, const Unit& u, int lane) {
+  bool ok = lane < u.sq.L;
+  if (p.mask_dtype == 1) ok = ok && u.mask_raw != 0;
+  if (p.mask_dtype == 2) ok = ok && __uint_as_float(static_cast<uint32_t>(u.mask_raw)) != 0.0f;
+  return __ballot_sync(0xffffffffu, ok);
 }
 
 template <int DH>
@@ -216,11 +247,6 @@
   }
 }
 
-A4R_DEVICE uint32_t build_keymask(const AttnParams& p, const SeqSpan& sq, int lane) {
-  const bool ok = lane < sq.L ? key_valid(p, sq, lane) : false;
-  return __ballot_sync(0xffffffffu, ok);
-}
-
 A4R_DEVICE void acc_to_a(uint32_t (&a)[4], const float (&c0)[4], const float (&c1)[4]) {
   a[0] = pack_bf16x2(c0[0], c0[1]);
   a[1] = pack_bf16x2(c0[2], c0[3]);
@@ -228,29 +254,52 @@
   a[3] = pack_bf16x2(c1[2], c1[3]);
 }
 
-template <int DH>
-__global__ void __launch_bounds__(WARPS_PER_CTA * 32, 3) attn_fwd_kernel(const AttnParams p) {
+constexpr int FWD_WARPS = 4;
+#ifndef XBWD_NBUF
+#define XBWD_NBUF 2
+#define XBWD_WARPS 7
+#define XBWD_MINB 1
+#endif
+constexpr int BWD_NBUF = XBWD_NBUF, BWD_WARPS = XBWD_WARPS;
+
+template <int DH>
+__host__ __device__ constexpr int fwd_warp_bytes() { return 3 * Tile<DH>::kBytes; }
+template <int DH>
+__host__ __device__ constexpr bool bwd_p_in_v() { return 2 * Tile<32>::kBytes <= Tile<DH>::kBytes; }
+template <int DH>
+__host__ __device__ constexpr int bwd_warp_bytes() { return BWD_NBUF * 4 * Tile<DH>::kBytes + (bwd_p_in_v<DH>() ? 0 : 2 * Tile<32>::kBytes); }
+
+template <int DH>
+A4R_DEVICE void load_qkv(uint8_t* buf, const AttnParams& p, const Unit& u, int q_rows, int lane) {
+  constexpr int TB = Tile<DH>::kBytes;
+  const int64_t Hd = static_cast<int64_t>(p.heads) * DH;
+  const __nv_bfloat16* q = p.qkv + u.sq.row0 * p.ld_qkv + u.h * DH;
+  load_tile<DH>(buf, q, p.ld_qkv, q_rows, lane);
+  load_tile<DH>(buf + TB, q + Hd, p.ld_qkv, u.sq.L, lane);
+  load_tile<DH>(buf + 2 * TB, q + 2 * Hd, p.ld_qkv, u.sq.L, lane);
+}
+A4R_DEVICE int64_t ctx_row0(const AttnParams& p, const Unit& u) { return p.cls_query ? u.n : u.sq.row0; }
+
+template <int DH>
+__global__ void __launch_bounds__(FWD_WARPS * 32, 3) attn_fwd_kernel(const AttnParams p) {
   extern __shared__ __align__(128) uint8_t smem_attn[];
   constexpr int TB = Tile<DH>::kBytes;
   const int warp = threadIdx.x >> 5, lane = threadIdx.x & 31;
-  uint8_t* my = smem_attn + warp * 3 * TB;
-  const int64_t total = static_cast<int64_t>(p.N) * p.heads;
-  for (int64_t w = static_cast<int64_t>(blockIdx.x) * WARPS_PER_CTA + warp; w < total;
-       w += static_cast<int64_t>(gridDim.x) * WARPS_PER_CTA) {
-    const int n = static_cast<int>(w / p.heads), h = static_cast<int>(w % p.heads);
-    const int64_t Hd = static_cast<int64_t>(p.heads) * DH;
-    const SeqSpan sq = seq_span(p, n);
-    const __nv_bfloat16* q = p.qkv + sq.row0 * p.ld_qkv + h * DH;
-    load_tile<DH>(my, q, p.ld_qkv, sq.L, lane);
-    load_tile<DH>(my + TB, q + Hd, p.ld_qkv, sq.L, lane);
-    load_tile<DH>(my + 2 * TB, q + 2 * Hd, p.ld_qkv, sq.L, lane);
-    const uint32_t km = build_keymask(p, sq, lane);
-    cp_async_wait_all();
-    __syncwarp();
-    const uint32_t sQ = smem_u32(my), sK = sQ + TB, sV = sK + TB;
+  uint8_t* my = smem_attn + warp * fwd_warp_bytes<DH>();
+  const uint32_t sQ = smem_u32(my), sK = sQ + TB, sV = sK + TB;
+  const int64_t total = static_cast<int64_t>(p.N) * p.heads, stride = static_cast<int64_t>(gridDim.x) * FWD_WARPS;
+  const uint64_t seed = p.drop_thr16 != 0 ? rng_seed(p.drop_seed) : 0;
+  for (int64_t w = static_cast<int64_t>(blockIdx.x) * FWD_WARPS + warp; w < total; w += stride) {
+    const Unit u = unit_at(p, w, lane);
+    load_qkv<DH>(my, p, u, p.cls_query ? 1 : u.sq.L, lane);
+    cp_async_commit();
+    const uint32_t keep = p.drop_thr16 != 0 ? prob_keep_bits(seed, p, u.n, u.h, lane) : 0u;
+    const uint32_t km = unit_keymask(p, u, lane);
+    cp_async_wait<0>();
+    __syncwarp();
     float s[2][4][4];
-    scores_softmax<DH>(s, sQ, sK, p, sq.L, lane, km);
-    if (p.drop_thr16 != 0) prob_dropout(s, p, n, h, lane);
+    scores_softmax<DH>(s, sQ, sK, p, u.sq.L, lane, km);
+    if (p.drop_thr16 != 0) prob_dropout(s, keep, p.drop_scale);
     float o[2][DH / 8][4];
 #pragma unroll
     for (int mt = 0; mt < 2; ++mt)
@@ -277,37 +326,55 @@
     __syncwarp();
     acc_to_tile<DH, DH / 8>(my, o, 1.f, 1.f, 1.f, 1.f, lane);
     __syncwarp();
-    store_tile<DH>(my, p.out + sq.row0 * p.ld_out + h * DH, p.ld_out, sq.L, lane);
-    __syncwarp();
-  }
-}
-
-template <int DH>
-__global__ void __launch_bounds__(WARPS_PER_CTA * 32) attn_bwd_kernel(const AttnParams p) {
+    store_tile<DH>(my, p.out + ctx_row0(p, u) * p.ld_out + u.h * DH, p.ld_out, p.cls_query ? 1 : u.sq.L, lane);
+    __syncwarp();
+  }
+}
+
+template <int DH>
+__global__ void __launch_bounds__(BWD_WARPS * 32, XBWD_MINB) attn_bwd_kernel(const AttnParams p) {
   extern __shared__ __align__(128) uint8_t smem_attn[];
   constexpr int TB = Tile<DH>::kBytes;
   constexpr int PB = Tile<32>::kBytes;
   const int warp = threadIdx.x >> 5, lane = threadIdx.x & 31;
-  uint8_t* my = smem_attn + warp * (4 * TB + 2 * PB);
-  const int64_t total = static_cast<int64_t>(p.N) * p.heads;
-  for (int64_t w = static_cast<int64_t>(blockIdx.x) * WARPS_PER_CTA + warp; w < total;
-       w += static_cast<int64_t>(gridDim.x) * WARPS_PER_CTA) {
-    const int n = static_cast<int>(w / p.heads), h = static_cast<int>(w % p.heads);
-    const int64_t Hd = static_cast<int64_t>(p.heads) * DH;
-    const SeqSpan sq = seq_span(p, n);
-    const __nv_bfloat16* q = p.qkv + sq.row0 * p.ld_qkv + h * DH;
-    uint8_t *tQ = my, *tK = my + TB, *tV = my + 2 * TB, *tdO = my + 3 * TB, *tP = my + 4 * TB, *tdS = tP + PB;
-    load_tile<DH>(tQ, q, p.ld_qkv, sq.L, lane);
-    load_tile<DH>(tK, q + Hd, p.ld_qkv, sq.L, lane);
-    load_tile<DH>(tV, q + 2 * Hd, p.ld_qkv, sq.L, lane);
-    load_tile<DH>(tdO, p.dout + sq.row0 * p.ld_out + h * DH, p.ld_out, sq.L, lane);
-    const uint32_t km = build_keymask(p, sq, lane);
-    cp_async_wait_all();
-    __syncwarp();
+  uint8_t* ring = smem_attn + warp * bwd_warp_bytes<DH>();
+  const int64_t total = static_cast<int64_t>(p.N) * p.heads, stride = static_cast<int64_t>(gridDim.x) * BWD_WARPS;
+  const int64_t Hd = static_cast<int64_t>(p.heads) * DH;
+  int64_t w = static_cast<int64_t>(blockIdx.x) * BWD_WARPS + warp;
+  if (w >= total) return;
+  const uint64_t seed = p.drop_thr16 != 0 ? rng_seed(p.drop_seed) : 0;
+  Unit u = unit_at(p, w, lane);
+  if (BWD_NBUF == 2) {
+    load_qkv<DH>(ring, p, u, u.sq.L, lane);
+    load_tile<DH>(ring + 3 * TB, p.dout + ctx_row0(p, u) * p.ld_out + u.h * DH, p.ld_out, p.cls_query ? 1 : u.sq.L, lane);
+    cp_async_commit();
+  }
+  for (int buf = 0;; buf ^= BWD_NBUF - 1) {
+    const int64_t wn = w + stride;
+    Unit un = u;
+    if (wn < total) un = unit_at(p, wn, lane);
+    if (BWD_NBUF == 2 && wn < total) {
+      uint8_t* nb = ring + (buf ^ 1) * 4 * TB;
+      load_qkv<DH>(nb, p, un, un.sq.L, lane);
+      load_tile<DH>(nb + 3 * TB, p.dout + ctx_row0(p, un) * p.ld_out + un.h * DH, p.ld_out, p.cls_query ? 1 : un.sq.L,
+                    lane);
+    }
+    if (BWD_NBUF == 1) {
+      load_qkv<DH>(ring, p, u, u.sq.L, lane);
+      load_tile<DH>(ring + 3 * TB, p.dout + ctx_row0(p, u) * p.ld_out + u.h * DH, p.ld_out, p.cls_query ? 1 : u.sq.L, lane);
+    }
+    cp_async_commit();
+    const uint32_t keep = p.drop_thr16 != 0 ? prob_keep_bits(seed, p, u.n, u.h, lane) : 0u;
+    const uint32_t km = unit_keymask(p, u, lane);
+    cp_async_wait<BWD_NBUF - 1>();
+    __syncwarp();
+    uint8_t *tQ = ring + buf * 4 * TB, *tK = tQ + TB, *tV = tQ + 2 * TB, *tdO = tQ + 3 * TB;
+    uint8_t* tP = bwd_p_in_v<DH>() ? tV : ring + BWD_NBUF * 4 * TB;
+    uint8_t* tdS = tP + PB;
     const uint32_t sQ = smem_u32(tQ), sK = smem_u32(tK), sV = smem_u32(tV), sdO = smem_u32(tdO), sP = smem_u32(tP),
                    sdS = smem_u32(tdS);
     float s[2][4][4];
-    scores_softmax<DH>(s, sQ, sK, p, sq.L, lane, km);
+    scores_softmax<DH>(s, sQ, sK, p, u.sq.L, lane, km);
     float dp[2][4][4];
 #pragma unroll
     for (int mt = 0; mt < 2; ++mt)
@@ -339,7 +406,7 @@
 #pragma unroll
         for (int e = 0; e < 4; ++e) sd[mt][nt][e] = s[mt][nt][e];
     if (p.drop_thr16 != 0) {
-      prob_dropout(sd, p, n, h, lane);
+      prob_dropout(sd, keep, p.drop_scale);
 #pragma unroll
       for (int mt = 0; mt < 2; ++mt)
 #pragma unroll
@@ -364,9 +431,11 @@
           for (int e = 0; e < 2; ++e)
             dp[mt][nt][hh * 2 + e] = s[mt][nt][hh * 2 + e] * (dp[mt][nt][hh * 2 + e] - d) * p.scale;
       }
+    __syncwarp();
     acc_to_tile<32, 4>(tP, sd, 1.f, 1.f, 1.f, 1.f, lane);
     acc_to_tile<32, 4>(tdS, dp, 1.f, 1.f, 1.f, 1.f, lane);
     __syncwarp();
+    __nv_bfloat16* dq = p.out + u.sq.row0 * p.ld_qkv + u.h * DH;
     float acc[2][DH / 8][4];
 #pragma unroll
     for (int mt = 0; mt < 2; ++mt)
@@ -390,48 +459,65 @@
         mma_bf16_16816(acc[1][np * 2 + 1], a1, b1);
       }
     }
-    float dk[2][DH / 8][4], dv[2][DH / 8][4];
+    __syncwarp();
+    acc_to_tile<DH, DH / 8>(tK, acc, 1.f, 1.f, 1.f, 1.f, lane);
+    __syncwarp();
+    store_tile<DH>(tK, dq, p.ld_qkv, u.sq.L, lane);
 #pragma unroll
     for (int mt = 0; mt < 2; ++mt)
 #pragma unroll
       for (int nt = 0; nt < DH / 8; ++nt)
 #pragma unroll
-        for (int e = 0; e < 4; ++e) dk[mt][nt][e] = dv[mt][nt][e] = 0.0f;
+        for (int e = 0; e < 4; ++e) acc[mt][nt][e] = 0.0f;
 #pragma unroll
     for (int ks = 0; ks < 2; ++ks) {
-      uint32_t a0[4], a1[4], p0[4], p1[4];
+      uint32_t a0[4], a1[4];
       load_a_t<32>(a0, sdS, 0, ks * 16, lane);
       load_a_t<32>(a1, sdS, 16, ks * 16, lane);
-      load_a_t<32>(p0, sP, 0, ks * 16, lane);
-      load_a_t<32>(p1, sP, 16, ks * 16, lane);
 #pragma unroll
       for (int np = 0; np < DH / 16; ++np) {
         uint32_t b[4];
         load_b_kn<DH>(b, sQ, np * 16, ks * 16, lane);
         const uint32_t b0[2] = {b[0], b[1]}, b1[2] = {b[2], b[3]};
-        mma_bf16_16816(dk[0][np * 2], a0, b0);
-        mma_bf16_16816(dk[0][np * 2 + 1], a0, b1);
-        mma_bf16_16816(dk[1][np * 2], a1, b0);
-        mma_bf16_16816(dk[1][np * 2 + 1], a1, b1);
+        mma_bf16_16816(acc[0][np * 2], a0, b0);
+        mma_bf16_16816(acc[0][np * 2 + 1], a0, b1);
+        mma_bf16_16816(acc[1][np * 2], a1, b0);
+        mma_bf16_16816(acc[1][np * 2 + 1], a1, b1);
+      }
+    }
+    __syncwarp();
+    acc_to_tile<DH, DH / 8>(tQ, acc, 1.f, 1.f, 1.f, 1.f, lane);
+    __syncwarp();
+    store_tile<DH>(tQ, dq + Hd, p.ld_qkv, u.sq.L, lane);
+#pragma unroll
+    for (int mt = 0; mt < 2; ++mt)
+#pragma unroll
+      for (int nt = 0; nt < DH / 8; ++nt)
+#pragma unroll
+        for (int e = 0; e < 4; ++e) acc[mt][nt][e] = 0.0f;
+#pragma unroll
+    for (int ks = 0; ks < 2; ++ks) {
+      uint32_t p0[4], p1[4];
+      load_a_t<32>(p0, sP, 0, ks * 16, lane);
+      load_a_t<32>(p1, sP, 16, ks * 16, lane);
+#pragma unroll
+      for (int np = 0; np < DH / 16; ++np) {
         uint32_t c[4];
         load_b_kn<DH>(c, sdO, np * 16, ks * 16, lane);
         const uint32_t c0[2] = {c[0], c[1]}, c1[2] = {c[2], c[3]};
-        mma_bf16_16816(dv[0][np * 2], p0, c0);
-        mma_bf16_16816(dv[0][np * 2 + 1], p0, c1);
-        mma_bf16_16816(dv[1][np * 2], p1, c0);
-        mma_bf16_16816(dv[1][np * 2 + 1], p1, c1);
-      }
-    }
-    __syncwarp();
-    acc_to_tile<DH, DH / 8>(tQ, acc, 1.f, 1.f, 1.f, 1.f, lane);
-    acc_to_tile<DH, DH / 8>(tK, dk, 1.f, 1.f, 1.f, 1.f, lane);
-    acc_to_tile<DH, DH / 8>(tV, dv, 1.f, 1.f, 1.f, 1.f, lane);
-    __syncwarp();
-    __nv_bfloat16* dq = p.out + sq.row0 * p.ld_qkv + h * DH;
-    store_tile<DH>(tQ, dq, p.ld_qkv, sq.L, lane);
-    store_tile<DH>(tK, dq + Hd, p.ld_qkv, sq.L, lane);
-    store_tile<DH>(tV, dq + 2 * Hd, p.ld_qkv, sq.L, lane);
-    __syncwarp();
+        mma_bf16_16816(acc[0][np * 2], p0, c0);
+        mma_bf16_16816(acc[0][np * 2 + 1], p0, c1);
+        mma_bf16_16816(acc[1][np * 2], p1, c0);
+        mma_bf16_16816(acc[1][np * 2 + 1], p1, c1);
+      }
+    }
+    __syncwarp();
+    acc_to_tile<DH, DH / 8>(tdO, acc, 1.f, 1.f, 1.f, 1.f, lane);
+    __syncwarp();
+    store_tile<DH>(tdO, dq + 2 * Hd, p.ld_qkv, u.sq.L, lane);
+    __syncwarp();
+    if (wn >= total) break;
+    w = wn, u = un;
   }
 }
 
@@ -448,6 +534,8 @@
   if (a->mask_dtype != 0)
     A4R_CHECK_ARG(a->mask != nullptr && (a->cu_seqlens != nullptr || a->mask_ld >= a->L), "attention: bad mask/mask_ld");
   A4R_CHECK_ARG(a->dropout_p >= 0.0f && a->dropout_p < 1.0f, "attention: dropout_p must be in [0,1)");
+  A4R_CHECK_ARG(a->cls_query_only == 0 || (a->cls_query_only == 1 && a->cu_seqlens == nullptr),
+                "attention_small: cls_query_only must be 0 or 1, and 0 with cu_seqlens");
   return a4r_device_check();
 }
 
@@ -472,20 +560,24 @@
   p.drop_scale = 65536.0f / static_cast<float>(65536u - p.drop_thr16);
   p.drop_seed = a->dropout_seed;
   p.drop_offset = a->dropout_offset;
+  p.cls_query = a->cls_query_only;
   return p;
 }
 
 template <typename K>
-int launch(K kernel, int smem, const AttnParams& p, cudaStream_t stream, bool* attr_done) {
-  if (!*attr_done) {
+int launch(K kernel, int warps, int smem, const AttnParams& p, cudaStream_t stream, int* ctas_per_sm) {
+  if (*ctas_per_sm == 0) {
     A4R_CUDA_OK(cudaFuncSetAttribute(kernel, cudaFuncAttributeMaxDynamicSharedMemorySize, smem));
-    *attr_done = true;
+    int n = 0;
+    A4R_CUDA_OK(cudaOccupancyMaxActiveBlocksPerMultiprocessor(&n, kernel, warps * 32, smem));
+    A4R_CHECK_ARG(n >= 1, "attention_small: kernel does not fit on an SM");
+    *ctas_per_sm = n;
   }
   const int64_t total = static_cast<int64_t>(p.N) * p.heads;
-  int64_t blocks = (total + WARPS_PER_CTA - 1) / WARPS_PER_CTA;
-  const int64_t cap = static_cast<int64_t>(a4r_num_sms()) * 8;
+  int64_t blocks = (total + warps - 1) / warps;
+  const int64_t cap = static_cast<int64_t>(a4r_num_sms()) * *ctas_per_sm;
   if (blocks > cap) blocks = cap;
-  kernel<<<static_cast<int>(blocks), WARPS_PER_CTA * 32, smem, stream>>>(p);
+  kernel<<<static_cast<int>(blocks), warps * 32, smem, stream>>>(p);
   A4R_LAUNCH_OK();
   a4r_count_launch(1);
   return A4R_OK;
@@ -498,10 +590,11 @@
   if (rc != A4R_OK) return rc;
   if (a->N == 0) return A4R_OK;
   const AttnParams p = to_params(a);
-  static bool done64 = false, done32 = false;
+  const cudaStream_t s = static_cast<cudaStream_t>(stream);
+  static int ctas64 = 0, ctas32 = 0;
   if (a->head_dim == 64)
-    return launch(attn_fwd_kernel<64>, WARPS_PER_CTA * 3 * Tile<64>::kBytes, p, static_cast<cudaStream_t>(stream), &done64);
-  return launch(attn_fwd_kernel<32>, WARPS_PER_CTA * 3 * Tile<32>::kBytes, p, static_cast<cudaStream_t>(stream), &done32);
+    return launch(attn_fwd_kernel<64>, FWD_WARPS, FWD_WARPS * fwd_warp_bytes<64>(), p, s, &ctas64);
+  return launch(attn_fwd_kernel<32>, FWD_WARPS, FWD_WARPS * fwd_warp_bytes<32>(), p, s, &ctas32);
 }
 
 extern "C" int a4r_attn_small_bwd(const a4r_attn_args* a, a4r_stream_t stream) {
@@ -510,10 +603,9 @@
   A4R_CHECK_ARG(a->dout != nullptr && a4r_aligned16(a->dout), "attention bwd: dout missing or unaligned");
   if (a->N == 0) return A4R_OK;
   const AttnParams p = to_params(a);
-  static bool done64 = false, done32 = false;
+  const cudaStream_t s = static_cast<cudaStream_t>(stream);
+  static int ctas64 = 0, ctas32 = 0;
   if (a->head_dim == 64)
-    return launch(attn_bwd_kernel<64>, WARPS_PER_CTA * (4 * Tile<64>::kBytes + 2 * Tile<32>::kBytes), p,
-                  static_cast<cudaStream_t>(stream), &done64);
-  return launch(attn_bwd_kernel<32>, WARPS_PER_CTA * (4 * Tile<32>::kBytes + 2 * Tile<32>::kBytes), p,
-                static_cast<cudaStream_t>(stream), &done32);
-}
+    return launch(attn_bwd_kernel<64>, BWD_WARPS, BWD_WARPS * bwd_warp_bytes<64>(), p, s, &ctas64);
+  return launch(attn_bwd_kernel<32>, BWD_WARPS, BWD_WARPS * bwd_warp_bytes<32>(), p, s, &ctas32);
+}
diff --git a/adapter4rec_b200/functional.py b/adapter4rec_b200/functional.py
--- a/adapter4rec_b200/functional.py
+++ b/adapter4rec_b200/functional.py
@@ -302,30 +302,33 @@
 
 class AttentionFunction(torch.autograd.Function):
     @staticmethod
-    def forward(ctx, qkv, mask, N, L, heads, head_dim, causal, mask_neg, dropout_p=0.0, scale=None, cu_seqlens=None):
-        ctx.cfg = (N, L, heads, head_dim, causal, mask_neg, scale)
+    def forward(ctx, qkv, mask, N, L, heads, head_dim, causal, mask_neg, dropout_p=0.0, scale=None, cu_seqlens=None,
+                cls_only=False):
+        ctx.cfg = (N, L, heads, head_dim, causal, mask_neg, scale, cls_only)
         ctx.cu = cu_seqlens
         ctx.mask = mask
         ctx.drop = None
         if dropout_p > 0.0:
             ctx.drop = (dropout_p,) + DropoutState.draw(N * heads * 32 * 8)
         out, lse = ops.attn_small_fwd(qkv, N, L, heads, head_dim, mask=mask, causal=causal, mask_neg=mask_neg, want_lse=True,
-                                      dropout=ctx.drop, scale=scale, cu_seqlens=cu_seqlens)
+                                      dropout=ctx.drop, scale=scale, cu_seqlens=cu_seqlens, cls_only=cls_only)
         ctx.save_for_backward(qkv, lse, out if lse is not None else None)
         return out
 
     @staticmethod
     def backward(ctx, dctx):
         qkv, lse, out = ctx.saved_tensors
-        N, L, heads, head_dim, causal, mask_neg, scale = ctx.cfg
+        N, L, heads, head_dim, causal, mask_neg, scale, cls_only = ctx.cfg
         dqkv = ops.attn_small_bwd(qkv, dctx.contiguous(), N, L, heads, head_dim, mask=ctx.mask, causal=causal,
-                                  mask_neg=mask_neg, lse=lse, ctx=out, dropout=ctx.drop, scale=scale, cu_seqlens=ctx.cu)
-        return dqkv, None, None, None, None, None, None, None, None, None, None
+                                  mask_neg=mask_neg, lse=lse, ctx=out, dropout=ctx.drop, scale=scale, cu_seqlens=ctx.cu,
+                                  cls_only=cls_only)
+        return dqkv, None, None, None, None, None, None, None, None, None, None, None
 
 
 def attention(qkv, mask, N, L, heads, head_dim, causal=False, mask_neg=ops.F32_MIN, dropout_p=0.0, scale=None,
-              cu_seqlens=None):
-    return AttentionFunction.apply(qkv, mask, N, L, heads, head_dim, causal, mask_neg, float(dropout_p), scale, cu_seqlens)
+              cu_seqlens=None, cls_only=False):
+    return AttentionFunction.apply(qkv, mask, N, L, heads, head_dim, causal, mask_neg, float(dropout_p), scale, cu_seqlens,
+                                   bool(cls_only))
 
 
 class GatherRowsFunction(torch.autograd.Function):
diff --git a/adapter4rec_b200/lib.py b/adapter4rec_b200/lib.py
--- a/adapter4rec_b200/lib.py
+++ b/adapter4rec_b200/lib.py
@@ -30,7 +30,7 @@
         ("mask_dtype", c_int32), ("causal", c_int32), ("scale", c_float), ("mask_neg", c_float),
         ("lse", c_void_p), ("ctx", c_void_p),
         ("dropout_p", c_float), ("dropout_seed", ctypes.c_uint64), ("dropout_offset", ctypes.c_uint64),
-        ("cu_seqlens", c_void_p),
+        ("cu_seqlens", c_void_p), ("cls_query_only", c_int32),
     ]
 
 
diff --git a/adapter4rec_b200/model/bert.py b/adapter4rec_b200/model/bert.py
--- a/adapter4rec_b200/model/bert.py
+++ b/adapter4rec_b200/model/bert.py
@@ -74,7 +74,7 @@
         self.dropout = nn.Dropout(config.attention_probs_dropout_prob)
         self._qkv_cache = {}
 
-    def forward(self, x2d, attention_mask, N, L, packed=None, want_skip=False):
+    def forward(self, x2d, attention_mask, N, L, packed=None, want_skip=False, cls_only=False):
         params = []
         for m in (self.query, self.key, self.value):
             params += [m.weight, m.bias, getattr(m, "lora_A", None), getattr(m, "lora_B", None)]
@@ -89,7 +89,8 @@
                                cu_seqlens=packed.cu_seqlens)
         else:
             ctx = Fn.attention(qkv, attention_mask, N, L, self.num_attention_heads, self.attention_head_size,
-                               causal=False, mask_neg=ops.F32_MIN, dropout_p=self.dropout.p if self.training else 0.0)
+                               causal=False, mask_neg=ops.F32_MIN, dropout_p=self.dropout.p if self.training else 0.0,
+                               cls_only=cls_only)
         return (ctx, skip) if want_skip else ctx
 
 
@@ -152,11 +153,12 @@
     def forward(self, x2d, attention_mask, N, L, cls_only=False, packed=None):
         if cls_only:
             H = x2d.shape[1]
-            ctx, skip = self.attention.self(x2d, attention_mask, N, L, packed, want_skip=True)
             if packed is not None:
+                ctx, skip = self.attention.self(x2d, attention_mask, N, L, packed, want_skip=True)
                 y = self.attention.output(Fn.gather_rows(ctx, packed.cls_rows), Fn.gather_rows(skip, packed.cls_rows))
             else:
-                y = self.attention.output(ctx.view(N, L, H)[:, 0], skip.view(N, L, H)[:, 0])
+                ctx, skip = self.attention.self(x2d, attention_mask, N, L, want_skip=True, cls_only=True)
+                y = self.attention.output(ctx, skip.view(N, L, H)[:, 0])
         else:
             y = self.attention(x2d, attention_mask, N, L, packed)
         out = self.output
diff --git a/adapter4rec_b200/ops.py b/adapter4rec_b200/ops.py
--- a/adapter4rec_b200/ops.py
+++ b/adapter4rec_b200/ops.py
@@ -148,11 +148,12 @@
 
 
 def attn_small_fwd(qkv, N, L, heads, head_dim, mask=None, causal=False, mask_neg=F32_MIN, want_lse=False, dropout=None,
-                   scale=None, cu_seqlens=None):
+                   scale=None, cu_seqlens=None, cls_only=False):
     assert qkv.dtype == BF16 and (cu_seqlens is not None or qkv.shape[0] == N * L)
-    out = torch.empty((qkv.shape[0], heads * head_dim), dtype=BF16, device=qkv.device)
+    assert not cls_only or (L <= 32 and cu_seqlens is None), "cls_only: short-sequence kernel, fixed-length layout"
+    out = torch.empty((N if cls_only else qkv.shape[0], heads * head_dim), dtype=BF16, device=qkv.device)
     a = _attn_args(qkv, N, L, heads, head_dim, mask, causal, mask_neg, dropout, scale, cu_seqlens)
-    a.out, a.ld_out = _p(out), out.stride(0)
+    a.out, a.ld_out, a.cls_query_only = _p(out), out.stride(0), int(cls_only)
     lse = None
     if want_lse and L > 32:
         lse = torch.empty((N * L, heads), dtype=torch.float32, device=qkv.device)
@@ -163,13 +164,14 @@
 
 
 def attn_small_bwd(qkv, dctx, N, L, heads, head_dim, mask=None, causal=False, mask_neg=F32_MIN, lse=None, ctx=None,
-                   dropout=None, scale=None, cu_seqlens=None):
-    assert qkv.dtype == BF16 and dctx.dtype == BF16 and dctx.shape[0] == qkv.shape[0]
+                   dropout=None, scale=None, cu_seqlens=None, cls_only=False):
+    assert qkv.dtype == BF16 and dctx.dtype == BF16 and dctx.shape[0] == (N if cls_only else qkv.shape[0])
     assert cu_seqlens is not None or qkv.shape[0] == N * L
+    assert not cls_only or (L <= 32 and cu_seqlens is None), "cls_only: short-sequence kernel, fixed-length layout"
     dqkv = torch.empty((qkv.shape[0], 3 * heads * head_dim), dtype=BF16, device=qkv.device)
     a = _attn_args(qkv, N, L, heads, head_dim, mask, causal, mask_neg, dropout, scale, cu_seqlens)
     assert _rows2d(qkv, "qkv") == dqkv.stride(0), "attention bwd expects a contiguous qkv"
-    a.out, a.dout, a.ld_out = _p(dqkv), _p(dctx), _rows2d(dctx, "dctx")
+    a.out, a.dout, a.ld_out, a.cls_query_only = _p(dqkv), _p(dctx), _rows2d(dctx, "dctx"), int(cls_only)
     if L > 32:
         assert lse is not None and ctx is not None and ctx.is_contiguous() and dctx.is_contiguous()
         a.lse, a.ctx = _p(lse), _p(ctx)
diff --git a/include/adapter4rec.h b/include/adapter4rec.h
--- a/include/adapter4rec.h
+++ b/include/adapter4rec.h
@@ -80,6 +80,7 @@
   uint64_t dropout_seed;
   uint64_t dropout_offset;
   const int32_t* cu_seqlens;
+  int32_t cls_query_only;
 } a4r_attn_args;
 
 A4R_API int a4r_attn_small_fwd(const a4r_attn_args* args, a4r_stream_t stream);
```

New measurement: 1952, median of 6. Within noise of the previous version (+0.2%).
